# nerfstudio-project/gsplat

Measured on AMD Instinct MI355X. Metric: Mpixels/s fwd+bwd @1M Gaussians/1080p, higher is better.
Workload: dtype f32; 1 GPU; c3: 1M synthetic Gaussians, 1x1920x1080, SH deg 3, 16x16 tiles, fwd+bwd; gaussians_per_gpu=1000000, cameras_per_gpu=1, packed=False, parallelism=single

## Files before the change

gsplat_amd/_autograd.py:

```python
from __future__ import annotations

import torch

from . import _ops

NS = _ops.NS
_registered = False


def _bwd(name):
    return _ops.impl(name + "_bwd")


def _cg(v):
    return None if v is None else v.contiguous()


def _z(v, shape, like):
    return like.new_zeros(shape) if v is None else v


def _qs_setup(ctx, inputs, output):
    quats, scales, compute_covar, compute_preci, triu = inputs
    ctx.triu = triu
    ctx.save_for_backward(quats, scales)


def _qs_backward(ctx, v_covars, v_precis):
    quats, scales = ctx.saved_tensors
    if v_covars is not None and v_covars.is_sparse:
        v_covars = v_covars.to_dense()
    if v_precis is not None and v_precis.is_sparse:
        v_precis = v_precis.to_dense()
    v_quats, v_scales = _bwd("quat_scale_to_covar_preci")(
        quats, scales, ctx.triu,
        None if v_covars is None else v_covars.contiguous(),
        None if v_precis is None else v_precis.contiguous(),
    )
    return v_quats, v_scales, None, None, None


def _sh_setup(ctx, inputs, output):
    (degrees_to_use, means, viewmats, coeffs, masks, batch_ids, camera_ids, gaussian_ids, viewmats_rs) = inputs
    ctx.degrees_to_use = degrees_to_use
    ctx.save_for_backward(means, viewmats, coeffs, masks, batch_ids, camera_ids, gaussian_ids, viewmats_rs)


def _sh_backward(ctx, v_colors):
    means, viewmats, coeffs, masks, batch_ids, camera_ids, gaussian_ids, viewmats_rs = ctx.saved_tensors
    v_coeffs, v_means, v_viewmats, v_viewmats_rs = _bwd("spherical_harmonics")(
        ctx.degrees_to_use, means, viewmats, coeffs, masks, batch_ids, camera_ids, gaussian_ids, viewmats_rs,
        v_colors.contiguous(), ctx.needs_input_grad[1], ctx.needs_input_grad[2],
        len(ctx.needs_input_grad) > 8 and ctx.needs_input_grad[8],
    )
    return (None, v_means, v_viewmats, v_coeffs, None, None, None, None, v_viewmats_rs)


def _proj_setup(ctx, inputs, output):
    (means, covars, quats, scales, _opacities, viewmats, Ks, width, height, eps2d, _near, _far, _clip, _calc,
     camera_model) = inputs
    radii, _means2d, _depths, conics, compensations = output
    ctx.width, ctx.height, ctx.eps2d, ctx.camera_model = width, height, eps2d, camera_model
    ctx.set_materialize_grads(False)
    ctx.m2_shape = _means2d.shape
    ctx.save_for_backward(means, covars, quats, scales, viewmats, Ks, radii, conics, compensations)


def _proj_backward(ctx, v_radii, v_means2d, v_depths, v_conics, v_compensations, v_view_opacities=None):
    means, covars, quats, scales, viewmats, Ks, radii, conics, compensations = ctx.saved_tensors
    if v_compensations is not None:
        v_compensations = v_compensations.contiguous()
    res = _bwd("projection_ewa_3dgs_fused")(
        means, covars, quats, scales, viewmats, Ks, ctx.width, ctx.height, ctx.eps2d, ctx.camera_model, radii, conics,
        compensations, _z(v_means2d, ctx.m2_shape, conics), None if v_depths is None else v_depths.contiguous(),
        _z(v_conics, conics.shape, conics), v_compensations, ctx.needs_input_grad[5], _v_view_opacities=v_view_opacities,
    )
    v_means, v_covars, v_quats, v_scales, v_viewmats = res[:5]
    v_opacities = res[5] if v_view_opacities is not None else None
    if not ctx.needs_input_grad[0]:
        v_means = None
    if not ctx.needs_input_grad[1]:
        v_covars = None
    if not ctx.needs_input_grad[2]:
        v_quats = None
    if not ctx.needs_input_grad[3]:
        v_scales = None
    return (v_means, v_covars, v_quats, v_scales, v_opacities, v_viewmats) + (None,) * 9


class ProjectionWithViewOpacities(torch.autograd.Function):

    @staticmethod
    def forward(ctx, *args):
        with torch._C._AutoDispatchBelowAutograd():
            out = getattr(torch.ops, NS).projection_ewa_3dgs_fused.default(*args)
        _proj_setup(ctx, args, out)
        opacities, viewmats = args[4], args[5]
        per_view = torch.broadcast_to(opacities[..., None, :], opacities.shape[:-1] + (viewmats.shape[-3], opacities.shape[-1]))
        per_view = per_view.contiguous()
        ctx.mark_non_differentiable(out[0])
        return tuple(out) + (per_view,)

    @staticmethod
    def backward(ctx, v_radii, v_means2d, v_depths, v_conics, v_compensations, v_per_view):
        if not ctx.needs_input_grad[4]:
            v_per_view = None
        return _proj_backward(ctx, v_radii, v_means2d, v_depths, v_conics, v_compensations, v_per_view)


def _projp_setup(ctx, inputs, output):
    (means, covars, quats, scales, _opacities, viewmats, Ks, width, height, eps2d, _near, _far, _clip, sparse_grad,
     _calc, camera_model) = inputs
    (batch_ids, camera_ids, gaussian_ids, _indptr, _radii, _means2d, _depths, conics, compensations) = output
    ctx.width, ctx.height, ctx.eps2d, ctx.camera_model, ctx.sparse_grad = width, height, eps2d, camera_model, sparse_grad
    ctx.set_materialize_grads(False)
    ctx.m2_shape = _means2d.shape
    ctx.save_for_backward(means, covars, quats, scales, viewmats, Ks, batch_ids, camera_ids, gaussian_ids, conics,
                          compensations)


def _projp_backward(ctx, v_batch_ids, v_camera_ids, v_gaussian_ids, v_indptr, v_radii, v_means2d, v_depths, v_conics,
                    v_compensations, v_view_opacities=None):
    (means, covars, quats, scales, viewmats, Ks, batch_ids, camera_ids, gaussian_ids, conics,
     compensations) = ctx.saved_tensors
    if v_compensations is not None:
        v_compensations = v_compensations.contiguous()
    res = _bwd("projection_ewa_3dgs_packed")(
        means, covars, quats, scales, viewmats, Ks, ctx.width, ctx.height, ctx.eps2d, ctx.camera_model,
        ctx.sparse_grad, batch_ids, camera_ids, gaussian_ids, conics, compensations,
        _z(v_means2d, ctx.m2_shape, conics), None if v_depths is None else v_depths.contiguous(),
        _z(v_conics, conics.shape, conics), v_compensations, ctx.needs_input_grad[5], _v_view_opacities=v_view_opacities,
    )
    v_means, v_covars, v_quats, v_scales, v_viewmats = res[:5]
    v_opacities = res[5] if v_view_opacities is not None else None
    if not ctx.needs_input_grad[0]:
        v_means = None
    if not ctx.needs_input_grad[1]:
        v_covars = None
    if not ctx.needs_input_grad[2]:
        v_quats = None
    if not ctx.needs_input_grad[3]:
        v_scales = None
    return (v_means, v_covars, v_quats, v_scales, v_opacities, v_viewmats) + (None,) * 10


class PackedProjectionWithViewOpacities(torch.autograd.Function):

    @staticmethod
    def forward(ctx, *args):
        with torch._C._AutoDispatchBelowAutograd():
            out = getattr(torch.ops, NS).projection_ewa_3dgs_packed.default(*args)
        _projp_setup(ctx, args, out)
        opacities = args[4]
        batch_ids, gaussian_ids = out[0], out[2]
        N = opacities.shape[-1]
        flat_ids = gaussian_ids if opacities.dim() == 1 else batch_ids * N + gaussian_ids
        row_opacities = opacities.reshape(-1).index_select(0, flat_ids)
        ctx.mark_non_differentiable(*[t for t in out[:5] if t is not None])
        return tuple(out) + (row_opacities,)

    @staticmethod
    def backward(ctx, v_b, v_c, v_g, v_indptr, v_radii, v_means2d, v_depths, v_conics, v_compensations, v_row_opacities):
        if not ctx.needs_input_grad[4]:
            v_row_opacities = None
        return _projp_backward(ctx, v_b, v_c, v_g, v_indptr, v_radii, v_means2d, v_depths, v_conics, v_compensations,
                               v_row_opacities)


def _rast_setup(ctx, inputs, output):
    (means2d, conics, colors, opacities, backgrounds, masks, image_width, image_height, tile_size, isect_offsets,
     flatten_ids, _packed, absgrad) = inputs
    _render_colors, render_alphas, means2d_absgrad, last_ids = output
    ctx.mark_non_differentiable(last_ids, means2d_absgrad)
    ctx.width, ctx.height, ctx.tile_size, ctx.absgrad = image_width, image_height, tile_size, absgrad
    ctx.set_materialize_grads(False)
    ctx.rc_shape = _render_colors.shape
    ctx.longest = _ops._lookup_longest(flatten_ids)
    ctx.save_for_backward(means2d, conics, colors, opacities, backgrounds, masks, isect_offsets, flatten_ids,
                          render_alphas, last_ids, means2d_absgrad)


def _rast_backward(ctx, v_render_colors, v_render_alphas, v_means2d_absgrad, v_last_ids):
    (means2d, conics, colors, opacities, backgrounds, masks, isect_offsets, flatten_ids, render_alphas, last_ids,
     means2d_absgrad) = ctx.saved_tensors
    v_means2d_abs, v_means2d, v_conics, v_colors, v_opacities, v_backgrounds = _bwd("rasterize_to_pixels_3dgs")(
        means2d, conics, colors, opacities, backgrounds, masks, isect_offsets, flatten_ids, render_alphas, last_ids,
        ctx.width, ctx.height, ctx.tile_size, ctx.absgrad, _z(v_render_colors, ctx.rc_shape, render_alphas),
        None if v_render_alphas is None else v_render_alphas.contiguous(), ctx.needs_input_grad[4], _longest=ctx.longest,
    )
    if ctx.absgrad and v_means2d_abs is not None:
        means2d_absgrad.copy_(v_means2d_abs)
    return (v_means2d, v_conics, v_colors, v_opacities, v_backgrounds) + (None,) * 8


def _rsp_setup(ctx, inputs, output):
    (means2d, conics, colors, opacities, backgrounds, masks, image_ids, image_width, image_height, tile_size, tile_width,
     tile_height, active_tiles, tile_offsets, flatten_ids, tile_pixel_mask, tile_pixel_cumsum, pixel_map, _packed,
     absgrad) = inputs
    _render_colors, render_alphas, means2d_absgrad, last_ids = output
    ctx.mark_non_differentiable(last_ids, means2d_absgrad)
    ctx.geom = (image_width, image_height, tile_size, tile_width, tile_height)
    ctx.absgrad = absgrad
    ctx.set_materialize_grads(False)
    ctx.rc_shape = _render_colors.shape
    ctx.save_for_backward(means2d, conics, colors, opacities, backgrounds, masks, image_ids, active_tiles, tile_offsets,
                          flatten_ids, tile_pixel_mask, tile_pixel_cumsum, pixel_map, render_alphas, last_ids,
                          means2d_absgrad)


def _rsp_backward(ctx, v_render_colors, v_render_alphas, v_means2d_absgrad, v_last_ids):
    (means2d, conics, colors, opacities, backgrounds, masks, image_ids, active_tiles, tile_offsets, flatten_ids,
     tile_pixel_mask, tile_pixel_cumsum, pixel_map, render_alphas, last_ids, means2d_absgrad) = ctx.saved_tensors
    v_means2d_abs, v_means2d, v_conics, v_colors, v_opacities, v_backgrounds = _bwd("rasterize_to_pixels_sparse")(
        means2d, conics, colors, opacities, backgrounds, masks, image_ids, active_tiles, tile_offsets, flatten_ids,
        tile_pixel_mask, tile_pixel_cumsum, pixel_map, render_alphas, last_ids, *ctx.geom, ctx.absgrad,
        _z(v_render_colors, ctx.rc_shape, render_alphas).contiguous(),
        None if v_render_alphas is None else v_render_alphas.contiguous(), ctx.needs_input_grad[4],
    )
    if ctx.absgrad and v_means2d_abs is not None:
        means2d_absgrad.copy_(v_means2d_abs)
    return (v_means2d, v_conics, v_colors, v_opacities, v_backgrounds) + (None,) * 15


def _p2_setup(ctx, inputs, output):
    means, quats, scales, viewmats, Ks, width, height, _eps2d, _near, _far, _clip = inputs
    radii, _means2d, _depths, ray_transforms, _normals = output
    ctx.width, ctx.height = width, height
    ctx.save_for_backward(means, quats, scales, viewmats, Ks, radii, ray_transforms)


def _p2_backward(ctx, v_radii, v_means2d, v_depths, v_ray_transforms, v_normals, v_view_opacities=None):
    means, quats, scales, viewmats, Ks, radii, ray_transforms = ctx.saved_tensors
    res = _bwd("projection_2dgs_fused")(
        means, quats, scales, viewmats, Ks, ctx.width, ctx.height, radii, ray_transforms, v_means2d,
        v_depths, v_ray_transforms, v_normals, ctx.needs_input_grad[3],
        _v_view_opacities=v_view_opacities)
    if v_view_opacities is not None:
        return tuple(res[:4]) + (None,) * 7 + (res[4],)
    return tuple(res) + (None,) * 7


class Projection2DGSWithViewOpacities(torch.autograd.Function):

    @staticmethod
    def forward(ctx, *args):
        op_args, opacities = args[:-1], args[-1]
        with torch._C._AutoDispatchBelowAutograd():
            out = getattr(torch.ops, NS).projection_2dgs_fused.default(*op_args)
        _p2_setup(ctx, op_args, out)
        viewmats = op_args[3]
        per_view = torch.broadcast_to(opacities[..., None, :], opacities.shape[:-1] + (viewmats.shape[-3], opacities.shape[-1]))
        per_view = per_view.contiguous()
        ctx.mark_non_differentiable(out[0])
        return tuple(out) + (per_view,)

    @staticmethod
    def backward(ctx, v_radii, v_means2d, v_depths, v_ray_transforms, v_normals, v_per_view):
        if v_per_view is None or not ctx.needs_input_grad[11]:
            return _p2_backward(ctx, v_radii, v_means2d, v_depths, v_ray_transforms, v_normals) + (None,)
        return _p2_backward(ctx, v_radii, v_means2d, v_depths, v_ray_transforms, v_normals, v_per_view)


def _p2p_setup(ctx, inputs, output):
    means, quats, scales, viewmats, Ks, width, height, _near, _far, _clip, sparse_grad = inputs
    batch_ids, camera_ids, gaussian_ids, _indptr, _radii, _means2d, _depths, ray_transforms, _normals = output
    ctx.width, ctx.height, ctx.sparse_grad = width, height, sparse_grad
    ctx.save_for_backward(means, quats, scales, viewmats, Ks, batch_ids, camera_ids, gaussian_ids, ray_transforms)


def _p2p_backward(ctx, v_b, v_c, v_g, v_indptr, v_radii, v_means2d, v_depths, v_ray_transforms, v_normals):
    means, quats, scales, viewmats, Ks, batch_ids, camera_ids, gaussian_ids, ray_transforms = ctx.saved_tensors
    v_means, v_quats, v_scales, v_viewmats = _bwd("projection_2dgs_packed")(
        means, quats, scales, viewmats, Ks, ctx.width, ctx.height, ctx.sparse_grad, batch_ids, camera_ids,
        gaussian_ids, ray_transforms, v_means2d, v_depths.contiguous(), v_ray_transforms, v_normals,
        ctx.needs_input_grad[3])
    return (v_means, v_quats, v_scales, v_viewmats) + (None,) * 7


def _r2_setup(ctx, inputs, output):
    (means2d, ray_transforms, colors, opacities, normals, densify, backgrounds, masks, image_width, image_height,
     tile_size, tile_offsets, flatten_ids, _packed, absgrad, _distloss) = inputs
    (render_colors, render_alphas, _rn, _rd, _rm, means2d_absgrad, last_ids, median_ids) = output
    ctx.mark_non_differentiable(last_ids, median_ids, means2d_absgrad)
    ctx.width, ctx.height, ctx.tile_size, ctx.absgrad = image_width, image_height, tile_size, absgrad
    ctx.set_materialize_grads(False)
    ctx.rc_shape = render_colors.shape
    ctx.save_for_backward(means2d, ray_transforms, colors, opacities, normals, densify, backgrounds, masks,
                          tile_offsets, flatten_ids, render_colors, render_alphas, last_ids, median_ids,
                          means2d_absgrad)


def _r2_backward(ctx, v_render_colors, v_render_alphas, v_render_normals, v_render_distort, v_render_median,
                 v_absgrad, v_last_ids, v_median_ids):
    (means2d, ray_transforms, colors, opacities, normals, densify, backgrounds, masks, tile_offsets, flatten_ids,
     render_colors, render_alphas, last_ids, median_ids, means2d_absgrad) = ctx.saved_tensors
    (v_means2d_abs, v_means2d, v_ray_transforms, v_colors, v_opacities, v_normals, v_densify,
     v_backgrounds) = _bwd("rasterize_to_pixels_2dgs")(
        means2d, ray_transforms, colors, opacities, normals, densify, backgrounds, masks, tile_offsets, flatten_ids,
        render_colors, render_alphas, last_ids, median_ids, ctx.width, ctx.height, ctx.tile_size, ctx.absgrad,
        _z(v_render_colors, ctx.rc_shape, render_alphas).contiguous(), _cg(v_render_alphas), _cg(v_render_normals),
        _cg(v_render_distort), _cg(v_render_median), ctx.needs_input_grad[6])
    if ctx.absgrad and v_means2d_abs is not None:
        means2d_absgrad.copy_(v_means2d_abs)
    return (v_means2d, v_ray_transforms, v_colors, v_opacities, v_normals, v_densify, v_backgrounds) + (None,) * 9


def _l0_setup(ctx, inputs, output):
    ctx.save_for_backward(inputs[0])


def _l0_backward(ctx, v_colors):
    (sh0,) = ctx.saved_tensors
    return _bwd("spherical_harmonics_l0")(sh0, v_colors.contiguous())


def _l1_setup(ctx, inputs, output):
    (degrees_to_use, means, viewmats, shN, masks, batch_ids, camera_ids, gaussian_ids, viewmats_rs) = inputs
    ctx.degrees_to_use = degrees_to_use
    ctx.save_for_backward(means, viewmats, shN, masks, batch_ids, camera_ids, gaussian_ids, viewmats_rs)


def _l1_backward(ctx, v_colors):
    means, viewmats, shN, masks, batch_ids, camera_ids, gaussian_ids, viewmats_rs = ctx.saved_tensors
    v_shN, v_means, v_viewmats, v_rs = _bwd("spherical_harmonics_l1_plus")(
        ctx.degrees_to_use, means, viewmats, shN, masks, batch_ids, camera_ids, gaussian_ids, viewmats_rs,
        v_colors.contiguous(), ctx.needs_input_grad[1], ctx.needs_input_grad[2],
        len(ctx.needs_input_grad) > 8 and ctx.needs_input_grad[8])
    return (None, v_means, v_viewmats, v_shN, None, None, None, None, v_rs)


def _simple_setup(ctx, inputs, output):
    means, covars, Ks, width, height, camera_model = inputs
    ctx.width, ctx.height, ctx.camera_model = width, height, camera_model
    ctx.save_for_backward(means, covars, Ks)


def _simple_backward(ctx, v_means2d, v_covars2d):
    means, covars, Ks = ctx.saved_tensors
    v_means, v_covars = _bwd("projection_ewa_simple")(means, covars, Ks, ctx.width, ctx.height, ctx.camera_model,
                                                      v_means2d.contiguous(), v_covars2d.contiguous())
    return v_means, v_covars, None, None, None, None


_TABLE = {
    "spherical_harmonics_l0": (_l0_backward, _l0_setup),
    "spherical_harmonics_l1_plus": (_l1_backward, _l1_setup),
    "projection_ewa_simple": (_simple_backward, _simple_setup),
    "projection_2dgs_fused": (_p2_backward, _p2_setup),
    "projection_2dgs_packed": (_p2p_backward, _p2p_setup),
    "rasterize_to_pixels_2dgs": (_r2_backward, _r2_setup),
    "quat_scale_to_covar_preci": (_qs_backward, _qs_setup),
    "spherical_harmonics": (_sh_backward, _sh_setup),
    "projection_ewa_3dgs_fused": (_proj_backward, _proj_setup),
    "projection_ewa_3dgs_packed": (_projp_backward, _projp_setup),
    "rasterize_to_pixels_3dgs": (_rast_backward, _rast_setup),
    "rasterize_to_pixels_sparse": (_rsp_backward, _rsp_setup),
}


def register(extra=None) -> None:
    global _registered
    if _registered:
        return
    table = dict(_TABLE)
    if extra:
        table.update(extra)
    for name, (bwd, setup) in table.items():
        try:
            torch.library.register_autograd(f"{NS}::{name}", bwd, setup_context=setup)
        except RuntimeError as e:
            if "already" not in str(e).lower():
                raise
    _registered = True


register()


class _FastOps:

    def __init__(self, extra=None):
        self._table = dict(_TABLE)
        if extra:
            self._table.update(extra)
        self._ns = getattr(torch.ops, NS)

    def __getattr__(self, name):
        entry = self._table.get(name)
        op = getattr(self._ns, name)
        if entry is None:
            fn = op
        else:
            bwd, setup = entry
            overload = op.default

            class _Fn(torch.autograd.Function):
                @staticmethod
                def forward(ctx, *args):
                    with torch._C._AutoDispatchBelowAutograd():
                        out = overload(*args)
                    setup(ctx, args, out)
                    return out

                @staticmethod
                def backward(ctx, *grads):
                    return bwd(ctx, *grads)

            _Fn.__name__ = _Fn.__qualname__ = f"gsplat_{name}"
            fn = _Fn.apply
        setattr(self, name, fn)
        return fn


fast_ops = _FastOps()
```

gsplat_amd/_cabi.py:

```python
from __future__ import annotations

import ctypes
import json
import os
import threading
from typing import Optional

import torch

_HERE = os.path.dirname(os.path.abspath(__file__))
_LIB_ENV = "GSPLAT_AMD_LIB"


class GsplatAmdError(RuntimeError):
    pass


def lib_path() -> str:
    return os.environ.get(_LIB_ENV) or os.path.join(_HERE, "csrc", "libgsplat_amd.so")


def _load() -> ctypes.CDLL:
    path = lib_path()
    if not os.path.exists(path):
# ... 26 lines not shown
            for a in args.split(","):
                a = " ".join(a.split())
                if "*" in a:
                    codes.append("p")
                elif a.startswith("uint32_t"):
                    codes.append("u")
                elif a.startswith("int64_t"):
                    codes.append("l")
                elif a.startswith("float"):
                    codes.append("f")
                elif a.startswith("double"):
                    codes.append("d")
                elif a.startswith("int "):
                    codes.append("i")
                else:
                    raise ImportError(f"gsplat_amd: cannot parse argument '{a}' of {name} in {path}")
        sigs[name] = ({"int": "i", "int64_t": "l", "void *": "p", "void": "v"}.get(ret, "s"), codes)
    return sigs


_SIG_TABLE = os.path.join(_HERE, "csrc", "abi_signatures.json")


def _load_signatures():
    if os.path.exists(_HEADER):
        return _parse_header(_HEADER)
    if os.path.exists(_SIG_TABLE):
        with open(_SIG_TABLE) as f:
            return {k: (v[0], list(v[1])) for k, v in json.load(f).items()}
    raise ImportError(f"gsplat_amd: neither {_HEADER} nor {_SIG_TABLE} found; rebuild with __graft_entry__.build()")


def write_signature_table() -> str:
    with open(_SIG_TABLE, "w") as f:
        json.dump({k: [v[0], v[1]] for k, v in _parse_header(_HEADER).items()}, f)
    return _SIG_TABLE


SIGNATURES = _load_signatures()


def _bind():
    for name, (ret, codes) in SIGNATURES.items():
        fn = getattr(_lib, name)
        fn.restype = {"i": ctypes.c_int, "l": _L, "s": ctypes.c_char_p, "p": ctypes.c_void_p, "v": None}[ret]
        fn.argtypes = [_CODES[c] for c in codes]


_bind()

ABI_VERSION = _lib.gsx_version()
ARCH = _lib.gsx_arch().decode()


def exported_symbols():
    return list(SIGNATURES)


_tls = threading.local()


def ptr(t: Optional[torch.Tensor]):
    if t is None:
        return None
    if not t.is_cuda:
        raise GsplatAmdError(
            "gsplat_amd kernels only run on a ROCm device (got a CPU tensor); there is no CPU fallback"
        )
    if not t.is_contiguous():
        raise GsplatAmdError("gsplat_amd: tensor must be contiguous")
    _tls.dev = t.device.index
    return t.data_ptr()


def ptr_host(t: torch.Tensor):
    if t.is_cuda or not t.is_pinned():
        raise GsplatAmdError("gsplat_amd: expected a pinned host tensor")
    return t.data_ptr()


def ptr_strided(t: torch.Tensor):
    if not t.is_cuda:
        raise GsplatAmdError("gsplat_amd kernels only run on a ROCm device (got a CPU tensor); there is no CPU fallback")
    _tls.dev = t.device.index
    return t.data_ptr()


_raw_stream = getattr(torch._C, "_cuda_getCurrentRawStream", None)


def current_stream() -> int:
    if _raw_stream is not None:
        return _raw_stream(torch.cuda.current_device())
    return torch.cuda.current_stream().cuda_stream


_profile = None
_profile_only = None


def torch_lib_path() -> str:
    if os.environ.get("GSPLAT_AMD_TORCH_LIB"):
        return os.environ["GSPLAT_AMD_TORCH_LIB"]
    d, base = os.path.split(lib_path())
    if not (base.startswith("libgsplat_amd") and base.endswith(".so")):
        raise ImportError(f"gsplat_amd: {_LIB_ENV}={lib_path()} does not follow the naming rule libgsplat_amd*.so; set "
                          "GSPLAT_AMD_TORCH_LIB to the libgsplat_amd_torch*.so linked against it")
    return os.path.join(d, "libgsplat_amd_torch" + base[len("libgsplat_amd"):])


def check_single_kernel_library() -> None:
    with open("/proc/self/maps") as f:
        libs = {os.path.realpath(ln.split(None, 5)[5].strip()) for ln in f if len(ln.split(None, 5)) == 6}
    kernels = {p for p in libs if os.path.basename(p).startswith("libgsplat_amd") and "_torch" not in os.path.basename(p)}
    if kernels != {os.path.realpath(lib_path())}:
        raise ImportError(f"gsplat_amd: {torch_lib_path()} is linked against {sorted(kernels - {os.path.realpath(lib_path())})}, "
                          f"not {lib_path()}; build the matching torch library (tools/mkvariant.sh, make SUFFIX=... torch)")


_torch_lib = None


def torch_lib() -> ctypes.CDLL:
    global _torch_lib
    if _torch_lib is None:
        lib = ctypes.CDLL(torch_lib_path())
        lib.gsx_torch_seg_len.argtypes, lib.gsx_torch_seg_len.restype = [], ctypes.c_int64
        lib.gsx_torch_profile_begin.argtypes, lib.gsx_torch_profile_begin.restype = [ctypes.c_char_p], None
        lib.gsx_torch_profile_end.restype = ctypes.c_char_p
        _torch_lib = lib
    return _torch_lib


def profile_begin(only=None) -> None:
    global _profile, _profile_only
    _profile = []
    _profile_only = None if only is None else frozenset(only)
    torch_lib().gsx_torch_profile_begin(" ".join(sorted(_profile_only or ())).encode())


def profile_end() -> dict:
    global _profile
    rec, _profile = _profile or [], None
    torch.cuda.synchronize()
    out = {}
    for name, a, b in rec:
        out.setdefault(name, []).append(a.elapsed_time(b))
    for line in torch_lib().gsx_torch_profile_end().decode().splitlines():
        name, ms = line.split()
        out.setdefault(name, []).append(float(ms))
    return out


def call(name: str, *args) -> None:
    dev = getattr(_tls, "dev", None)
    if dev is not None and dev != torch.cuda.current_device():
        _tls.dev = None
        with torch.cuda.device(dev):
            return call(name, *args)
    fn = getattr(_lib, name)
    if _profile is not None and (_profile_only is None or name in _profile_only):
        a, b = torch.cuda.Event(enable_timing=True), torch.cuda.Event(enable_timing=True)
        a.record()
        rc = fn(*args, current_stream())
        b.record()
        _profile.append((name, a, b))
    else:
        rc = fn(*args, current_stream())
    if rc != 0:
        msg = _lib.gsx_last_error().decode(errors="replace")
        if rc == -1:
            raise ValueError(f"{name}: {msg}")
        raise GsplatAmdError(f"{name} failed (code {rc}): {msg}")


def scan_workspace_bytes(n: int) -> int:
    return int(_lib.gsx_scan_workspace_bytes(n))


def sort_workspace_bytes(n: int) -> int:
    return int(_lib.gsx_sort_pairs_workspace_bytes(n))


def appearance_bwd_workspace_floats(n: int, n_cameras: int) -> int:
    return int(_lib.gsx_appearance_bwd_workspace_floats(n, n_cameras))


def knn_workspace_bytes(n: int, k: int) -> int:
    return int(_lib.gsx_knn_workspace_bytes(n, k))


def kmeans_workspace_bytes(n: int, d: int, k: int) -> int:
    return int(_lib.gsx_kmeans_workspace_bytes(n, d, k))


def plas_workspace_bytes(h: int, w: int, c: int) -> int:
    return int(_lib.gsx_plas_workspace_bytes(h, w, c))


def plas_partials_floats(h: int, w: int) -> int:
    return int(_lib.gsx_plas_partials_floats(h, w))


def tile_sort_supported(n_images: int, tile_w: int, tile_h: int) -> bool:
    return bool(_lib.gsx_isect_tile_sort_supported(n_images, tile_w, tile_h))


def tile_sort_workspace_bytes(n: int, n_images: int, tile_w: int, tile_h: int) -> int:
    return int(_lib.gsx_isect_tile_sort_workspace_bytes(n, n_images, tile_w, tile_h))


def isect_fused_supported(n_images: int, tile_w: int, tile_h: int, packed: bool) -> bool:
    return bool(_lib.gsx_isect_fused_supported(n_images, tile_w, tile_h, int(packed)))


class IsectPathMemory:

    def __init__(self):
        self._h = _lib.gsx_isect_path_memory_create()
        if not self._h:
            raise MemoryError("gsx_isect_path_memory_create failed")
        self._prev = []

    def __enter__(self):
        self._prev.append(_lib.gsx_isect_path_memory_use(self._h))
        return self

    def __exit__(self, *exc):
        _lib.gsx_isect_path_memory_use(self._prev.pop())
        return False

    def __del__(self):
        h, self._h = getattr(self, "_h", None), None
        if h:
            _lib.gsx_isect_path_memory_destroy(h)


def copy_column_groups(groups, rows: int) -> None:
    n = len(groups)
    src = (ctypes.c_void_p * n)(*[g[0] for g in groups])
    dst = (ctypes.c_void_p * n)(*[g[2] for g in groups])
    ss = (ctypes.c_uint32 * n)(*[g[1] for g in groups])
    ds = (ctypes.c_uint32 * n)(*[g[3] for g in groups])
    w = (ctypes.c_uint32 * n)(*[g[4] for g in groups])
    call("gsx_copy_column_groups", n, src, ss, dst, ds, w, rows)


def copy_column_groups_mapped(groups, seg_rows, seg_n, map_dst: bool) -> None:
    n, m = len(groups), len(seg_rows)
    src = (ctypes.c_void_p * n)(*[g[0] for g in groups])
    dst = (ctypes.c_void_p * n)(*[g[2] for g in groups])
    ss = (ctypes.c_uint32 * n)(*[g[1] for g in groups])
    ds = (ctypes.c_uint32 * n)(*[g[3] for g in groups])
    w = (ctypes.c_uint32 * n)(*[g[4] for g in groups])
    sr = (ctypes.c_int64 * m)(*[int(v) for v in seg_rows])
    sn = (ctypes.c_int64 * m)(*[int(v) for v in seg_n])
    call("gsx_copy_column_groups_mapped", n, src, ss, dst, ds, w, m, sr, sn, int(bool(map_dst)))


def copy_message_columns(msg_ptr: int, msg_stride: int, rows: int, groups, to_message: bool, seg_rows=None, seg_n=None) -> None:
    n = len(groups)
    cols = (ctypes.c_uint32 * n)(*[g[0] for g in groups])
    w = (ctypes.c_uint32 * n)(*[g[1] for g in groups])
    fields = (ctypes.c_void_p * n)(*[g[2] for g in groups])
    fs = (ctypes.c_uint32 * n)(*[g[3] for g in groups])
    m = 0 if seg_rows is None else len(seg_rows)
    sr = (ctypes.c_int64 * max(m, 1))(*([int(v) for v in seg_rows] if m else [0]))
    sn = (ctypes.c_int64 * max(m, 1))(*([int(v) for v in seg_n] if m else [0]))
    call("gsx_copy_message_columns", ctypes.c_void_p(msg_ptr), msg_stride, rows, n, cols, w, fields, fs, int(bool(to_message)), m,
         sr, sn)


def sort_pairs(keys, vals, keys_alt, vals_alt, n: int, end_bit: int, workspace) -> bool:
    flag = ctypes.c_int(0)
    rc = _lib.gsx_sort_pairs(ptr(keys), ptr(vals), ptr(keys_alt), ptr(vals_alt), n, end_bit, ptr(workspace),
                             workspace.numel() * workspace.element_size(), ctypes.addressof(flag), current_stream())
    if rc != 0:
        raise GsplatAmdError(f"gsx_sort_pairs failed (code {rc}): {_lib.gsx_last_error().decode(errors='replace')}")
    return bool(flag.value)
```

gsplat_amd/_ops.py:

```python
from __future__ import annotations

import math
import os
import threading
from typing import Optional, Tuple

import torch
from torch import Tensor

from . import _cabi
from ._cabi import call, ptr, ptr_strided

NS = "gsplat"

_lib_def = torch.library.Library(NS, "FRAGMENT")
_lib_impl = torch.library.Library(NS, "IMPL", "CUDA")
_lib_impl_autograd = torch.library.Library(NS, "IMPL", "AutogradCUDA")


def _load_torch_lib() -> None:
    path = _cabi.torch_lib_path()
    hint = "build it with `make -C gsplat_amd/csrc torch`"
    if not os.path.exists(path):
        raise ImportError(f"gsplat_amd: {path} not found; {hint}")
# ... 578 lines not shown
         ptr(isect_ids), ptr(flatten_ids))
    if sort:
        isect_ids, flatten_ids = _sort_isects(isect_ids, flatten_ids, I, int(lidar.n_bins_azimuth), int(lidar.n_bins_elevation),
                                              32 + tile_bits + image_bits)
    return tiles_per_gauss, isect_ids, flatten_ids


def _proj_dims(means, viewmats):
    batch_dims = means.shape[:-2]
    return batch_dims, math.prod(batch_dims), viewmats.shape[-3], means.shape[-2]


def _f64_instantiation(fn):
    import functools

    @functools.wraps(fn)
    def body(means, *args, **kw):
        if means.dtype != torch.float64:
            return fn(means, *args, **kw)
        down = lambda t: t.to(torch.float32) if isinstance(t, Tensor) and t.dtype == torch.float64 else t
        up = lambda t: t.to(torch.float64) if isinstance(t, Tensor) and t.dtype == torch.float32 else t
        out = fn(down(means), *[down(a) for a in args], **{k: down(v) for k, v in kw.items()})
        return tuple(up(t) for t in out)

    return body


@_op("projection_ewa_3dgs_fused_bwd")
@_f64_instantiation
def projection_ewa_3dgs_fused_bwd(means, covars, quats, scales, viewmats, Ks, image_width, image_height, eps2d,
                                  camera_model, radii, conics, compensations, v_means2d, v_depths, v_conics,
                                  v_compensations, viewmats_requires_grad, *, _v_view_opacities=None):
    batch_dims, B, C, N = _proj_dims(means, viewmats)
    means, viewmats, Ks = means.contiguous(), viewmats.contiguous(), Ks.contiguous()
    covars, quats, scales = _c(covars), _c(quats), _c(scales)
    v_means = torch.empty_like(means)
    v_covars = v_quats = v_scales = None
    if covars is not None:
        v_covars = torch.empty_like(covars)
    else:
        v_quats, v_scales = torch.empty_like(quats), torch.empty_like(scales)
    v_viewmats = torch.zeros_like(viewmats) if viewmats_requires_grad else None
    v_means2d, m2_stride = _row_view(v_means2d, 2)
    v_conics, con_stride = _row_view(v_conics, 3)
    head = (ptr(means), ptr(covars), ptr(None if covars is not None else quats),
            ptr(None if covars is not None else scales), ptr(viewmats), ptr(Ks), B, C, N, image_width, image_height,
            eps2d, int(camera_model), ptr(radii.contiguous()), ptr(conics.contiguous()), ptr(_c(compensations)),
            ptr_strided(v_means2d), m2_stride, ptr(_c(v_depths)), ptr_strided(v_conics), con_stride,
            ptr(_c(v_compensations)))
    if _v_view_opacities is not None:
        v_view, opac_stride = _elem_view(_v_view_opacities)
        v_opacities = torch.empty(tuple(batch_dims) + (N,), device=means.device, dtype=means.dtype)
        call("gsx_project_ewa_bwd_opac", *head, ptr_strided(v_view), opac_stride, ptr(v_means), ptr(v_covars), ptr(v_quats),
             ptr(v_scales), ptr(v_viewmats), ptr(v_opacities))
        return v_means, v_covars, v_quats, v_scales, v_viewmats, v_opacities
    call("gsx_project_ewa_bwd", *head, ptr(v_means), ptr(v_covars), ptr(v_quats), ptr(v_scales), ptr(v_viewmats))
    return v_means, v_covars, v_quats, v_scales, v_viewmats


@_op("projection_ewa_3dgs_packed_bwd")
@_f64_instantiation
def projection_ewa_3dgs_packed_bwd(means, covars, quats, scales, viewmats, Ks, image_width, image_height, eps2d,
                                   camera_model, sparse_grad, batch_ids, camera_ids, gaussian_ids, conics,
                                   compensations, v_means2d, v_depths, v_conics, v_compensations,
                                   viewmats_requires_grad, *, _v_view_opacities=None):
    batch_dims, B, C, N = _proj_dims(means, viewmats)
    means, viewmats, Ks = means.contiguous(), viewmats.contiguous(), Ks.contiguous()
    covars, quats, scales = _c(covars), _c(quats), _c(scales)
    nnz = gaussian_ids.shape[0]
    v_viewmats = torch.zeros_like(viewmats) if viewmats_requires_grad else None
    v_means2d, m2_stride = _row_view(v_means2d, 2)
    v_conics, con_stride = _row_view(v_conics, 3)
    head = (ptr(means), ptr(covars), ptr(None if covars is not None else quats),
            ptr(None if covars is not None else scales), ptr(viewmats), ptr(Ks), B, C, N, image_width, image_height,
            eps2d, int(camera_model), nnz, ptr(batch_ids.contiguous()), ptr(camera_ids.contiguous()),
            ptr(gaussian_ids.contiguous()), ptr(conics.contiguous()), ptr(_c(compensations)),
            ptr_strided(v_means2d), m2_stride, ptr(_c(v_depths)), ptr_strided(v_conics), con_stride,
            ptr(_c(v_compensations)))
    def scatter_opacities():
        flat = torch.zeros(B * N, device=means.device, dtype=means.dtype)
        flat.index_add_(0, batch_ids * N + gaussian_ids if B > 1 else gaussian_ids, _v_view_opacities.reshape(-1))
        return flat.reshape(tuple(batch_dims) + (N,))

    if sparse_grad:
        def rows(width):
            return torch.empty((nnz, width), device=means.device, dtype=means.dtype)

        r_means = rows(3)
        r_covars = rows(6) if covars is not None else None
        r_quats = rows(4) if covars is None else None
        r_scales = rows(3) if covars is None else None
        call("gsx_project_ewa_packed_bwd_rows", *head, ptr(r_means), ptr(r_covars), ptr(r_quats), ptr(r_scales),
             ptr(v_viewmats))
        flat = len(batch_dims) == 0
        indices = gaussian_ids.unsqueeze(0) if flat else torch.stack([batch_ids, gaussian_ids])
        coalesced = B * C == 1

        def coo(vals, like):
            if vals is None:
                return None
            size = ((N,) if flat else (B, N)) + (like.shape[-1],)
            sp = torch.sparse_coo_tensor(indices, vals, size=size, is_coalesced=coalesced)
            return sp if len(batch_dims) <= 1 else sp.to_dense().reshape(like.shape)

        res = (coo(r_means, means), coo(r_covars, covars), coo(r_quats, quats), coo(r_scales, scales), v_viewmats)
        clear_row_map_cache()
        return res if _v_view_opacities is None else res + (scatter_opacities(),)
    gaussian_major = B * C > 1 or 2 * nnz >= N
    row_map = _packed_row_map(batch_ids, camera_ids, gaussian_ids, B, C, N) if (gaussian_major and nnz > 0 and N > 0) else None
    alloc = torch.empty_like if row_map is not None else torch.zeros_like
    v_means = alloc(means)
    v_covars = v_quats = v_scales = None
    if covars is not None:
        v_covars = alloc(covars)
    else:
        v_quats, v_scales = alloc(quats), alloc(scales)
    v_opacities = None
    if _v_view_opacities is not None:
        v_view, opac_stride = _elem_view(_v_view_opacities)
        v_opacities = (torch.empty if row_map is not None else torch.zeros)(tuple(batch_dims) + (N,), device=means.device, dtype=means.dtype)
        call("gsx_project_ewa_packed_bwd_opac", *head, ptr_strided(v_view), opac_stride, ptr(row_map), ptr(v_means), ptr(v_covars),
             ptr(v_quats), ptr(v_scales), ptr(v_viewmats), ptr(v_opacities))
    else:
        call("gsx_project_ewa_packed_bwd", *head, ptr(row_map), ptr(v_means), ptr(v_covars), ptr(v_quats), ptr(v_scales),
             ptr(v_viewmats))
    clear_row_map_cache()
    res = (v_means, v_covars, v_quats, v_scales, v_viewmats)
    return res if _v_view_opacities is None else res + (v_opacities,)


def _raster_dims(isect_offsets, colors):
    image_dims = tuple(isect_offsets.shape[:-2])
    return image_dims, math.prod(image_dims), isect_offsets.shape[-2], isect_offsets.shape[-1], colors.shape[-1]


def _pixel_linear_strides(t):
    if t.is_contiguous() or t.dim() < 3:
        return None
    shape, stride = t.shape, t.stride()
    cs, ps = stride[-1], stride[-2]
    if cs < 0 or ps < 0:
        return None
    expect = ps
    for d in range(t.dim() - 2, -1, -1):
        if shape[d] != 1 and stride[d] != expect:
            return None
        expect *= shape[d]
    return int(ps), int(cs)


@_op("rasterize_to_pixels_3dgs_bwd")
def rasterize_to_pixels_3dgs_bwd(means2d, conics, colors, opacities, backgrounds, masks, tile_offsets, flatten_ids,
                                 render_alphas, last_ids, image_width, image_height, tile_size, absgrad,
                                 v_render_colors, v_render_alphas, compute_v_backgrounds, *, _longest=None):
    image_dims, I, th, tw, D = _raster_dims(tile_offsets, colors)
    as_received = (means2d, conics, colors, opacities, tile_offsets, flatten_ids)
    means2d, conics, colors, opacities = (means2d.contiguous(), conics.contiguous(), colors.contiguous(),
                                          opacities.contiguous())
    backgrounds, masks = _c(backgrounds), _c(masks)
    v_render_alphas = _c(v_render_alphas)
    R = opacities.numel()
    geo = 8 if absgrad else 6
    longest = _longest if _longest is not None else _lookup_longest(flatten_ids)
    segmented = (longest > SEG_MIN_LONGEST and not absgrad and D <= 4 and tile_size == 16
                 and longest > _seg_cut(flatten_ids.numel(), I, tw, th))
    rows = (torch.zeros if segmented else torch.empty)((R, geo + D), device=means2d.device, dtype=means2d.dtype)
    vrc_strides = None if segmented else _pixel_linear_strides(v_render_colors)
    if vrc_strides is None:
        v_render_colors = v_render_colors.contiguous()
        vrc_strides = (-1, 1)
    if segmented:
        ws = torch.empty(_cabi._lib.gsx_raster3d_bwd_seg_workspace_bytes(flatten_ids.numel(), I, tw, th, D, SEG_LEN),
                         device=means2d.device, dtype=torch.uint8)
        fws = _lookup_seg_workspace(last_ids, flatten_ids.numel(), D, as_received)
        call("gsx_raster3d_bwd_seg_reuse", ptr(means2d), ptr(conics), ptr(colors), ptr(opacities), ptr(backgrounds), ptr(masks),
             ptr(tile_offsets.contiguous()), ptr(flatten_ids.contiguous()), ptr(render_alphas.contiguous()),
             ptr(last_ids.contiguous()), ptr(v_render_colors), ptr(v_render_alphas), I, flatten_ids.numel(), D,
             image_width, image_height, tile_size, tw, th, ptr(rows), geo + D, SEG_LEN, ptr(fws),
             0 if fws is None else fws.numel(), ptr(ws), ws.numel())
    else:
        ws = torch.empty(_cabi._lib.gsx_raster3d_bwd_workspace_bytes(I, tw, th), device=means2d.device, dtype=torch.uint8)
        call("gsx_raster3d_bwd_fill", ptr(means2d), ptr(conics), ptr(colors), ptr(opacities), ptr(backgrounds), ptr(masks),
             ptr(tile_offsets.contiguous()), ptr(flatten_ids.contiguous()), ptr(render_alphas.contiguous()),
             ptr(last_ids.contiguous()), ptr_strided(v_render_colors), ptr(v_render_alphas), I, flatten_ids.numel(), D,
             image_width, image_height, tile_size, tw, th, int(bool(absgrad)), ptr(rows), geo + D, R, vrc_strides[0],
             vrc_strides[1], ptr(ws), ws.numel())
    v_means2d, v_conics = rows[:, 0:2].view(means2d.shape), rows[:, 2:5].view(conics.shape)
    v_opacities, v_colors = rows[:, 5].view(opacities.shape), rows[:, geo:].view(colors.shape)
    v_abs = rows[:, 6:8].view(means2d.shape) if absgrad else None
    v_backgrounds = None
    if backgrounds is not None and compute_v_backgrounds:
        v_backgrounds = (v_render_colors * (1.0 - render_alphas)).sum(dim=(-3, -2))
    return v_abs, v_means2d, v_conics, v_colors, v_opacities, v_backgrounds


_SH_C0 = 0.2820947917738781


@_op("spherical_harmonics_l0")
def spherical_harmonics_l0(sh0):
    if sh0.dim() != 3:
        raise ValueError(f"sh0 must have shape [N, 1, D], got {tuple(sh0.shape)}")
    if sh0.shape[-2] != 1:
        raise ValueError(f"sh0 must contain exactly one SH coefficient, got {tuple(sh0.shape)}")
    if sh0.shape[-1] < 1:
        raise ValueError(f"sh0 last dim D must be >= 1, got {sh0.shape[-1]}")
    if sh0.dtype not in (torch.float32, torch.float16):
        raise TypeError(f"gsplat_amd: sh0 must be float32 or float16 (got {sh0.dtype})")
    return sh0[:, 0, :].float() * _SH_C0


@_op("spherical_harmonics_l0_bwd")
def spherical_harmonics_l0_bwd(sh0, v_colors):
    if v_colors.dim() != 2 or v_colors.shape[0] != sh0.shape[0] or v_colors.shape[1] != sh0.shape[2]:
        raise ValueError(f"v_colors must have shape [N, D], got {tuple(v_colors.shape)}")
    return (v_colors * _SH_C0)[:, None, :].to(sh0.dtype).contiguous()


def _pad_band0(shN):
    return torch.cat([torch.zeros_like(shN[:, :1]), shN], dim=1).contiguous()


_BAND_DTYPES = {torch.float32: 0, torch.float16: 1}


def _sh_band_fwd(degrees_to_use, first_band, means, viewmats, coeffs, masks, batch_ids, camera_ids, gaussian_ids):
    packed, B, C, N, KM, D = _sh_dims(means, viewmats, coeffs, gaussian_ids)
    means, viewmats, coeffs, masks = means.contiguous(), viewmats.contiguous(), coeffs.contiguous(), _c(masks)
    if coeffs.shape[0] != N:
        raise ValueError(f"coefficient rows are indexed by Gaussian: expected {N} rows, got {coeffs.shape[0]}")
    K = KM + first_band
    if packed:
        nnz = gaussian_ids.shape[0]
        colors = torch.empty((nnz, 3), device=means.device, dtype=means.dtype)
        call("gsx_sh_band_fwd", degrees_to_use, first_band, _BAND_DTYPES[coeffs.dtype], ptr(means), ptr(viewmats), ptr(coeffs),
             ptr(masks), ptr(_c(batch_ids)), ptr(_c(camera_ids)), ptr(_c(gaussian_ids)), B, C, N, nnz, K, ptr(colors))
    else:
        colors = torch.empty(viewmats.shape[:-2] + (N, 3), device=means.device, dtype=means.dtype)
        call("gsx_sh_band_fwd", degrees_to_use, first_band, _BAND_DTYPES[coeffs.dtype], ptr(means), ptr(viewmats), ptr(coeffs),
             ptr(masks), None, None, None, B, C, N, -1, K, ptr(colors))
    return colors


def _sh_band_bwd(degrees_to_use, first_band, means, viewmats, coeffs, masks, batch_ids, camera_ids, gaussian_ids, v_colors,
                 compute_v_means, compute_v_viewmats):
    packed, B, C, N, KM, D = _sh_dims(means, viewmats, coeffs, gaussian_ids)
    means, viewmats, coeffs, masks = means.contiguous(), viewmats.contiguous(), coeffs.contiguous(), _c(masks)
    K = KM + first_band
    nnz = gaussian_ids.shape[0] if packed else -1
    row_map = _packed_row_map(batch_ids, camera_ids, gaussian_ids, B, C, N) if (packed and nnz > 0 and N > 0) else None
    if packed and row_map is None:
        return torch.zeros_like(coeffs), (torch.zeros_like(means) if compute_v_means else None), \
            (torch.zeros_like(viewmats) if compute_v_viewmats else None)
    v_coeffs = torch.empty_like(coeffs)
    v_means = torch.empty_like(means) if compute_v_means else None
    v_dirs = None
    if compute_v_viewmats:
        v_dirs = torch.zeros(((nnz if packed else B * C * N), 3), device=means.device, dtype=means.dtype)
    call("gsx_sh_band_bwd", degrees_to_use, first_band, _BAND_DTYPES[coeffs.dtype], ptr(means), ptr(viewmats), ptr(coeffs),
         ptr(masks), B, C, N, nnz, K, ptr(v_colors.contiguous()), ptr(row_map), ptr(v_coeffs), ptr(v_means), ptr(v_dirs))
    v_viewmats = None
    if compute_v_viewmats:
        if packed:
            S = torch.zeros((B * C, 3), device=means.device, dtype=means.dtype)
            S.index_add_(0, batch_ids * C + camera_ids, v_dirs)
        else:
            S = v_dirs.view(B * C, N, 3).sum(dim=1)
        vm = viewmats.reshape(B * C, 4, 4)
        R, t = vm[:, :3, :3], vm[:, :3, 3]
        v_vm = torch.zeros_like(vm)
        v_vm[:, :3, :3] = t[:, :, None] * S[:, None, :]
        v_vm[:, :3, 3] = torch.einsum("cij,cj->ci", R, S)
        v_viewmats = v_vm.reshape(viewmats.shape)
    return v_coeffs, v_means, v_viewmats


def _band_kernels_apply(coeffs) -> bool:
    return coeffs.dim() == 3 and coeffs.shape[-1] == 3 and coeffs.shape[-2] >= 1 and coeffs.dtype in _BAND_DTYPES


@_op("spherical_harmonics_l1_plus")
def spherical_harmonics_l1_plus(degrees_to_use, means, viewmats, shN, masks, batch_ids, camera_ids, gaussian_ids,
                                viewmats_rs=None, *, _gathered: bool = True):
    if viewmats_rs is not None:
        viewmats = _sh_rs_viewmats(viewmats, viewmats_rs)
    if shN.dim() != 3:
        raise ValueError(f"shN must have shape [N, K - 1, D], got {tuple(shN.shape)}")
    _check_sh_inputs(degrees_to_use, means, viewmats, shN, masks, batch_ids, camera_ids, gaussian_ids, omit_l0=True,
                     gathered=_gathered)
    _check_f32(means=means, viewmats=viewmats)
    packed = gaussian_ids is not None
    if degrees_to_use == 0 or shN.shape[-2] == 0:
        shape = (shN.shape[0] if _gathered else gaussian_ids.shape[0], shN.shape[-1]) if packed \
            else tuple(viewmats.shape[:-2]) + (means.shape[-2], shN.shape[-1])
        return torch.zeros(shape, device=means.device, dtype=means.dtype)
    if _band_kernels_apply(shN) and not (packed and _gathered):
        return _sh_band_fwd(degrees_to_use, 1, means, viewmats, shN, masks, batch_ids, camera_ids, gaussian_ids)
    return spherical_harmonics(degrees_to_use, means, viewmats, _pad_band0(shN), masks, batch_ids, camera_ids,
                               gaussian_ids, None, _gathered=_gathered)


@_op("spherical_harmonics_l1_plus_bwd")
def spherical_harmonics_l1_plus_bwd(degrees_to_use, means, viewmats, shN, masks, batch_ids, camera_ids, gaussian_ids,
                                    viewmats_rs, v_colors, compute_v_means, compute_v_viewmats, compute_v_viewmats_rs,
                                    *, _gathered: bool = True):
    if viewmats_rs is not None:
        v_shN, v_me, v_syn, _ = spherical_harmonics_l1_plus_bwd(
            degrees_to_use, means, _sh_rs_viewmats(viewmats, viewmats_rs), shN, masks, batch_ids, camera_ids, gaussian_ids, None,
            v_colors, compute_v_means, compute_v_viewmats or compute_v_viewmats_rs, False, _gathered=_gathered)
        v_vm, v_rs = (None, None) if v_syn is None else _sh_rs_split(v_syn, viewmats, viewmats_rs, compute_v_viewmats,
                                                                     compute_v_viewmats_rs)
        return v_shN, v_me, v_vm, v_rs
    packed = gaussian_ids is not None
    if degrees_to_use == 0 or shN.shape[-2] == 0:
        return (torch.zeros_like(shN), torch.zeros_like(means) if compute_v_means else None,
                torch.zeros_like(viewmats) if compute_v_viewmats else None, None)
    if _band_kernels_apply(shN) and not (packed and _gathered):
        v_shN, v_means, v_viewmats = _sh_band_bwd(degrees_to_use, 1, means, viewmats, shN, masks, batch_ids, camera_ids,
                                                  gaussian_ids, v_colors, compute_v_means, compute_v_viewmats)
        return v_shN, v_means, v_viewmats, None
    v_coeffs, v_means, v_viewmats, v_rs = spherical_harmonics_bwd(
        degrees_to_use, means, viewmats, _pad_band0(shN), masks, batch_ids, camera_ids, gaussian_ids, viewmats_rs,
        v_colors, compute_v_means, compute_v_viewmats, compute_v_viewmats_rs, _gathered=_gathered)
    return v_coeffs[:, 1:].contiguous(), v_means, v_viewmats, v_rs


@_op("projection_ewa_simple")
def projection_ewa_simple(means, covars, Ks, width, height, camera_model):
    _check_f32(means=means, covars=covars, Ks=Ks)
    if means.shape[-1] != 3 or covars.shape[-2:] != (3, 3) or covars.shape[:-2] != means.shape[:-1]:
        raise ValueError(f"proj: bad shapes means {tuple(means.shape)} covars {tuple(covars.shape)}")
    means, covars, Ks = means.contiguous(), covars.contiguous(), Ks.contiguous()
    N = means.shape[-2]
    rows = means.numel() // 3
    means2d = torch.empty(means.shape[:-1] + (2,), device=means.device, dtype=means.dtype)
    covars2d = torch.empty(means.shape[:-1] + (2, 2), device=means.device, dtype=means.dtype)
    call("gsx_project_simple_fwd", ptr(means), ptr(covars), ptr(Ks), rows, N, width, height, int(camera_model),
         ptr(means2d), ptr(covars2d))
    return means2d, covars2d
# ... 1272 lines not shown
```

gsplat_amd/csrc/raster3d.hpp:

```cpp
#pragma once
#include "common.hpp"

#include <type_traits>

namespace gsx {

struct Raster3DArgs {
    uint32_t n_images;
    uint32_t n_isects;
    uint32_t width;
    uint32_t height;
    uint32_t tile_size;
    uint32_t tile_w;
    uint32_t tile_h;
    uint32_t cdim;
    uint32_t ch_off;
    uint32_t nch;
    uint32_t first_chunk;
    const float *means2d;
    const float *conics;
    const float *colors;
    const float *opacities;
    const float *backgrounds;
    const uint8_t *masks;
    const int32_t *isect_offsets;
    const int32_t *flatten_ids;
    float *render_colors;
    float *render_alphas;
    int32_t *last_ids;
    const float *v_render_colors;
    uint32_t vrc_strided;
    int64_t vrc_ps, vrc_cs;
    const float *v_render_alphas;
    float *v_rows;
    uint32_t row_stride;
    const int32_t *sp_active_tiles;
    const uint64_t *sp_pixel_mask;
    const int64_t *sp_pixel_cumsum;
    const int64_t *sp_pixel_map;
    uint32_t n_active, sp_words;
    uint32_t seg_mode, seg_len, seg_grid;
    uint32_t seg_cut;
    const int32_t *seg_items;
    const int32_t *seg_count;
    float *seg_T;
    float *seg_out;
    int32_t *seg_last;
    const int32_t *tile_order;
};

inline Raster3DArgs raster3d_args(uint32_t n_images, uint32_t n_isects, uint32_t cdim, uint32_t width, uint32_t height,
                                  uint32_t tile_size, uint32_t tile_w, uint32_t tile_h, const float *means2d, const float *conics,
                                  const float *colors, const float *opacities, const float *backgrounds, const uint8_t *masks,
                                  const int32_t *isect_offsets, const int32_t *flatten_ids, float *render_colors,
                                  const float *render_alphas, const int32_t *last_ids)
{
    Raster3DArgs a{};
    a.n_images = n_images; a.n_isects = n_isects; a.width = width; a.height = height;
    a.tile_size = tile_size; a.tile_w = tile_w; a.tile_h = tile_h; a.cdim = cdim;
    a.means2d = means2d; a.conics = conics; a.colors = colors; a.opacities = opacities;
    a.backgrounds = backgrounds; a.masks = masks; a.isect_offsets = isect_offsets; a.flatten_ids = flatten_ids;
    a.render_colors = render_colors; a.render_alphas = const_cast<float *>(render_alphas);
    a.last_ids = const_cast<int32_t *>(last_ids);
    return a;
}
inline void raster3d_set_bwd(Raster3DArgs &a, const float *v_render_colors, const float *v_render_alphas, float *v_rows,
                             uint32_t row_stride)
{
    a.v_render_colors = v_render_colors; a.v_render_alphas = v_render_alphas;
    a.v_rows = v_rows; a.row_stride = row_stride;
}
inline void raster3d_set_sparse(Raster3DArgs &a, const int32_t *active_tiles, const uint64_t *tile_pixel_mask,
                                const int64_t *tile_pixel_cumsum, const int64_t *pixel_map, uint32_t n_active,
                                uint32_t words_per_tile)
{
    a.sp_active_tiles = active_tiles; a.sp_pixel_mask = tile_pixel_mask; a.sp_pixel_cumsum = tile_pixel_cumsum;
    a.sp_pixel_map = pixel_map; a.n_active = n_active; a.sp_words = words_per_tile;
}

template <class F>
inline auto with_channels4(uint32_t n, F &&f)
{
    if (n <= 1) return f(std::integral_constant<int, 1>{});
    if (n <= 2) return f(std::integral_constant<int, 2>{});
    if (n <= 3) return f(std::integral_constant<int, 3>{});
    return f(std::integral_constant<int, 4>{});
}
template <class F>
inline auto with_channels(uint32_t n, F &&f)
{
    if (n <= 4) return with_channels4(n, f);
    if (n <= 8) return f(std::integral_constant<int, 8>{});
    if (n <= 16) return f(std::integral_constant<int, 16>{});
    return f(std::integral_constant<int, 32>{});
}

__device__ __forceinline__ uint32_t xcd_remap(uint32_t b, uint32_t n_blocks)
{
    constexpr uint32_t kXcds = 8;
    const uint32_t per_xcd   = (n_blocks + kXcds - 1) / kXcds;
    return (b % kXcds) * per_xcd + (b / kXcds);
}

template <typename Args>
__device__ __forceinline__ size_t vrc_index(const Args &a, size_t pix, uint32_t k)
{
    return a.vrc_strided ? (size_t)((int64_t)pix * a.vrc_ps + (int64_t)k * a.vrc_cs) : pix * a.cdim + k;
}

struct TileCtx {
    uint32_t image_id, tile_id, tile_x, tile_y;
    int32_t range_start, range_end;
};
template <class Args>
__device__ __forceinline__ bool tile_context(const Args &a, uint32_t block, TileCtx &t)
{
    const uint32_t tiles_per_image = a.tile_w * a.tile_h;
    if (a.sp_active_tiles) {
        const uint32_t at = xcd_remap(block, a.n_active);
        if (at >= a.n_active) return false;
        const uint32_t gt = (uint32_t)a.sp_active_tiles[at];
        t.image_id = gt / tiles_per_image;
        t.tile_id  = gt % tiles_per_image;
        t.range_start = a.isect_offsets[at];
        t.range_end   = a.isect_offsets[at + 1];
    } else {
        const uint32_t n_blocks = tiles_per_image * a.n_images;
        const uint32_t blk      = xcd_remap(block, n_blocks);
        if (blk >= n_blocks) return false;
        t.image_id = blk / tiles_per_image;
        t.tile_id  = blk % tiles_per_image;
        t.range_start = a.isect_offsets[blk];
        t.range_end   = (blk == n_blocks - 1) ? (int32_t)a.n_isects : a.isect_offsets[blk + 1];
    }
    t.tile_x = t.tile_id % a.tile_w;
    t.tile_y = t.tile_id / a.tile_w;
    return true;
}
__device__ __forceinline__ bool tile_context_seg(const Raster3DArgs &a, uint32_t block, TileCtx &t, uint32_t &item)
{
    item = 0;
    if (a.seg_mode == 0u) {
        if (!tile_context(a, block, t)) return false;
        return !(a.seg_len && !a.sp_active_tiles && (uint32_t)(t.range_end - t.range_start) > a.seg_cut);
    }
    const int32_t n_items = *a.seg_count;
    const uint32_t tiles_per_image = a.tile_w * a.tile_h, n_blocks = tiles_per_image * a.n_images;
    if ((int32_t)block >= n_items) {
        if (a.seg_mode != 2u) return false;
        const uint32_t blk = block - (uint32_t)n_items;
        if (blk >= n_blocks) return false;
        item       = 0xFFFFFFFFu;
        t.image_id = blk / tiles_per_image;
        t.tile_id  = blk % tiles_per_image;
        t.tile_x   = t.tile_id % a.tile_w;
        t.tile_y   = t.tile_id / a.tile_w;
        t.range_start = a.isect_offsets[blk];
        t.range_end   = (blk == n_blocks - 1) ? (int32_t)a.n_isects : a.isect_offsets[blk + 1];
        return (uint32_t)(t.range_end - t.range_start) <= a.seg_cut;
    }
    item = block;
    const uint32_t blk = (uint32_t)a.seg_items[2 * block];
    t.image_id = blk / tiles_per_image;
    t.tile_id  = blk % tiles_per_image;
    t.tile_x   = t.tile_id % a.tile_w;
    t.tile_y   = t.tile_id / a.tile_w;
    const int32_t tile_end = (blk == n_blocks - 1) ? (int32_t)a.n_isects : a.isect_offsets[blk + 1];
    t.range_start = a.seg_items[2 * block + 1];
    t.range_end   = min(t.range_start + (int32_t)a.seg_len, tile_end);
    return true;
}

template <class Args>
__device__ __forceinline__ int64_t pixel_row(const Args &a, const TileCtx &t, uint32_t block, uint32_t lx, uint32_t ly)
{
    if (!(lx < a.tile_size && ly < a.tile_size)) return -1;
    const uint32_t ox = t.tile_x * a.tile_size + lx, oy = t.tile_y * a.tile_size + ly;
    if (!(ox < a.width && oy < a.height)) return -1;
    if (!a.sp_active_tiles) return ((int64_t)t.image_id * a.height + oy) * a.width + ox;
    const uint32_t at      = xcd_remap(block, a.n_active);
    const uint64_t *words  = a.sp_pixel_mask + (size_t)at * a.sp_words;
    const uint32_t in_tile = ly * a.tile_size + lx, word = in_tile >> 6, bit = in_tile & 63u;
    if (!((words[word] >> bit) & 1ull)) return -1;
    uint32_t rank = __popcll(words[word] & ((1ull << bit) - 1ull));
    for (uint32_t w = 0; w < word; ++w) rank += __popcll(words[w]);
    const int64_t first = at == 0 ? 0 : a.sp_pixel_cumsum[at - 1];
    return a.sp_pixel_map[first + rank];
}

int64_t tile_order_workspace_bytes(uint32_t n_images, uint32_t tile_w, uint32_t tile_h);
const int32_t *build_tile_order(const int32_t *isect_offsets, const int32_t *last_ids, uint32_t n_images, uint32_t tile_size,
                                uint32_t tile_w, uint32_t tile_h, uint32_t width, uint32_t height, uint32_t n_isects, void *ws,
                                int64_t ws_bytes, hipStream_t stream, int *rc, void *zero_ptr = nullptr, int64_t zero_bytes = 0);

struct RowFill {
    const char *fn;
    float *rows;
    int64_t bytes;
    hipStream_t stream;
    template <class Args>
    const int32_t *tile_order(const Args &a, void *ws, int64_t ws_bytes, int *rc)
    {
        const bool in_kernel = bytes > 0 && (reinterpret_cast<uintptr_t>(rows) & 15u) == 0;
        const int32_t *order = build_tile_order(a.isect_offsets, a.last_ids, a.n_images, a.tile_size, a.tile_w, a.tile_h, a.width,
                                                a.height, a.n_isects, ws, ws_bytes, stream, rc, in_kernel ? rows : nullptr, bytes);
        if (*rc == GSX_OK && order && in_kernel) bytes = 0;
        return order;
    }
    int now()
    {
        if (bytes > 0 && rows && hipMemsetAsync(rows, 0, (size_t)bytes, stream) != hipSuccess) {
            set_last_error("%s: memset failed", fn);
            return GSX_ERR_LAUNCH;
        }
        bytes = 0;
        return GSX_OK;
    }
};

bool raster3d_fwd_m_applies(const Raster3DArgs &a);
int raster3d_fwd_m_launch(const Raster3DArgs &a, hipStream_t stream);

__device__ __forceinline__ bool tile_context_ordered(const Raster3DArgs &a, uint32_t block, TileCtx &t)
{
    const uint32_t tiles_per_image = a.tile_w * a.tile_h, n_blocks = tiles_per_image * a.n_images;
    const uint32_t idx = xcd_remap(block, n_blocks);
    if (idx >= n_blocks) return false;
    const uint32_t blk = (uint32_t)a.tile_order[idx];
    t.image_id = blk / tiles_per_image;
    t.tile_id  = blk % tiles_per_image;
    t.tile_x   = t.tile_id % a.tile_w;
    t.tile_y   = t.tile_id / a.tile_w;
    t.range_start = a.isect_offsets[blk];
    t.range_end   = (blk == n_blocks - 1) ? (int32_t)a.n_isects : a.isect_offsets[blk + 1];
    return true;
}

enum class BwdKernel { R, T, W, M };
BwdKernel raster3d_bwd_kernel(uint32_t tile_size, uint32_t nch, bool has_abs);
int raster3d_bwd_m_launch(const Raster3DArgs &a, hipStream_t stream);

__device__ __forceinline__ void tile_pixel(uint32_t tid, uint32_t tile_size, uint32_t &lx, uint32_t &ly)
{
    if (tile_size == 16) {
        const uint32_t w = tid >> 6, l = tid & 63u;
        lx = ((w & 1u) << 3) | (l & 7u);
        ly = ((w >> 1) << 3) | (l >> 3);
    } else {
        lx = tid % tile_size;
        ly = tid / tile_size;
    }
}

constexpr float kLog2e = 1.4426950408889634f;
__device__ __forceinline__ void stage_gaussian(float x, float y, float opac, float ca, float cb, float cc, float4 &ga,
                                               float2 &gb)
{
    const float lo = opac > 0.0f ? __log2f(opac) : -INFINITY;
    ga = make_float4(x, y, lo, 0.5f * kLog2e * ca);
    gb = make_float2(kLog2e * cb, 0.5f * kLog2e * cc);
}
__device__ __forceinline__ float staged_q(const float4 &ga, const float2 &gb, float dx, float dy)
{
    return fmaf(dx, fmaf(ga.w, dx, gb.x * dy), gb.y * dy * dy);
}
__device__ __forceinline__ float staged_alpha_raw(const float4 &ga, float q)
{
    return __builtin_amdgcn_exp2f(ga.z - q);
}
__device__ __forceinline__ float staged_e_offset(const float4 &ga, const float2 &gb, float dx, float dy)
{
    return fmaf(dx, fmaf(-gb.x, dy, -ga.w * dx), fmaf(-gb.y * dy, dy, ga.z));
}

struct StagedRow {
    v4f p0;
    v4f p1;
    v4f p2;
};
__device__ __forceinline__ void stage_gaussian_f(float ax, float ay, float opac, float ca, float cb, float cc, v4f &p0,
                                                 float &nA, float &nB, float &nC)
{
    const float lo = opac > 0.0f ? __log2f(opac) : -INFINITY;
    p0 = v4f{ax, ay, lo, lo};
    nA = -0.5f * kLog2e * ca; nB = -kLog2e * cb; nC = -0.5f * kLog2e * cc;
}
__device__ __forceinline__ float staged_f(const v4f &p0, float nA, float nB, float nC, float u, float v)
{
    const float dx = p0.x - u, dy = p0.y - v;
    return fmaf(dx, fmaf(nB, dy, nA * dx), fmaf(nC * dy, dy, p0.z));
}

__device__ __forceinline__ float2 cull_half_extent(float opac, float ca, float cb, float cc)
{
    const float L   = __logf(255.0f * opac) + 0.01f;
    const float det = ca * cc - cb * cb;
    if (!(det > 0.0f)) return make_float2(INFINITY, INFINITY);
    if (!(L > 0.0f)) return make_float2(-1.0f, -1.0f);
    const float k = 2.0f * L / det;
    return make_float2(sqrtf(k * cc) * 1.0001f + 1e-3f, sqrtf(k * ca) * 1.0001f + 1e-3f);
}

struct WaveRect {
    float cx, cy, hw, hh;
    bool any;
};
__device__ __forceinline__ WaveRect wave_pixel_rect(bool inside, float px, float py)
{
    float xmin = inside ? px : INFINITY, xmax = inside ? px : -INFINITY;
    float ymin = inside ? py : INFINITY, ymax = inside ? py : -INFINITY;
#pragma unroll
    for (int o = 32; o >= 1; o >>= 1) {
        xmin = fminf(xmin, __shfl_xor(xmin, o));
        xmax = fmaxf(xmax, __shfl_xor(xmax, o));
        ymin = fminf(ymin, __shfl_xor(ymin, o));
        ymax = fmaxf(ymax, __shfl_xor(ymax, o));
    }
    WaveRect r;
    r.any = xmin <= xmax;
    r.cx = 0.5f * (xmin + xmax); r.hw = 0.5f * (xmax - xmin);
    r.cy = 0.5f * (ymin + ymax); r.hh = 0.5f * (ymax - ymin);
    return r;
}

__device__ __forceinline__ bool rect_reaches_level(const v4f &p0, const v4f &p1, float ax, float ay, const WaveRect &r)
{
    const float A = -p1.x, B = -p1.y, C = -p1.z;
    if (!(A > 0.0f && C > 0.0f && 4.0f * A * C > B * B)) return true;
    const float dxl = ax - r.cx - r.hw, dxh = ax - r.cx + r.hw, dyl = ay - r.cy - r.hh, dyh = ay - r.cy + r.hh;
    const float dxe = fminf(fmaxf(0.0f, dxl), dxh), dye = fminf(fmaxf(0.0f, dyl), dyh);
    const float dys = fminf(fmaxf(-0.5f * B * dxe * __builtin_amdgcn_rcpf(C), dyl), dyh);
    const float dxs = fminf(fmaxf(-0.5f * B * dye * __builtin_amdgcn_rcpf(A), dxl), dxh);
    const float q1 = fmaf(dxe, fmaf(A, dxe, B * dys), C * dys * dys);
    const float q2 = fmaf(dxs, fmaf(A, dxs, B * dye), C * dye * dye);
    return fminf(q1, q2) <= p0.w + (7.99435344f + 0.01f);
}

}
```

gsplat_amd/csrc/raster3d_bwd.hip:

```cpp
#include <cstdlib>

#include "raster3d.hpp"
#include "../../include/gsplat_amd.h"

namespace gsx {

template <int CH, bool ABS>
struct BwdCfg {
    static constexpr int K     = CH + 6 + (ABS ? 2 : 0);
    static constexpr bool TAIL1 = (K % 4) == 1;
    static constexpr int KQ    = TAIL1 ? K / 4 : (K + 3) / 4;
    static constexpr int KP    = (K | 1);
    static constexpr int BATCH = (CH >= 16) ? 128 : 256;
    static constexpr size_t smem =
        (size_t)BATCH * (2 * sizeof(float4) + sizeof(float2) + sizeof(int32_t) * 2 + sizeof(float) * (CH + KP));
};

template <int CH, bool ABS>
__global__ void __launch_bounds__(256) raster3d_bwd_kernel(const Raster3DArgs a)
{
    using Cfg           = BwdCfg<CH, ABS>;
    constexpr int K     = Cfg::K;
    constexpr int KQ    = Cfg::KQ;
    constexpr int KP    = Cfg::KP;
// ... 827 lines not shown
                contributed |= 1 << q;
            }
            if (contributed) {
                const int info = (t << 4) | contributed;
                uint32_t m0_saved;
                asm("s_mov_b32 %1, m0\n\ts_mov_b32 m0, %3\n\tv_writelane_b32 %0, %2, m0\n\ts_mov_b32 m0, %1"
                    : "+v"(slot_info), "=&s"(m0_saved)
                    : "s"(info), "s"(slot));
                w_ptr += SP;
                if (++slot == SLOTS) {
                    turn(SLOTS);
                    slot  = 0;
                    w_ptr = w_ptr0;
                }
            }
        }
        if (slot) {
            turn(slot);
            slot  = 0;
            w_ptr = w_ptr0;
        }
    }
}

template <int CH>
__global__ void __launch_bounds__(64) __attribute__((amdgpu_waves_per_eu(GSX_BWD_W_WAVES)))
raster3d_bwd_w_kernel(Raster3DArgs a)
{
    raster3d_bwd_w_body<CH, false>(a);
}
__global__ void __launch_bounds__(64) __attribute__((amdgpu_waves_per_eu(2))) raster3d_bwd_w4_kernel(Raster3DArgs a)
{
    raster3d_bwd_w_body<4, false>(a);
}
template <int CH>
__global__ void __launch_bounds__(64) __attribute__((amdgpu_waves_per_eu(GSX_BWD_W_ABS_WAVES)))
raster3d_bwd_w_abs_kernel(Raster3DArgs a)
{
    raster3d_bwd_w_body<CH, true>(a);
}

BwdKernel raster3d_bwd_kernel(uint32_t tile_size, uint32_t nch, bool has_abs)
{
    static const char v = [] {
        const char *e = getenv("GSX_RASTER3D_BWD");
        if (e && (e[0] == 'r' || e[0] == 'R')) return 'r';
        if (e && (e[0] == 't' || e[0] == 'T')) return 't';
        return 'w';
    }();
    if (tile_size != 16 || v == 'r') return BwdKernel::R;
    if (nch > 4) return !has_abs && nch <= 32 ? BwdKernel::M : BwdKernel::R;
    if (v == 'w') return BwdKernel::W;
    return has_abs ? BwdKernel::R : BwdKernel::T;
}

template <int CH, bool ABS>
static int launch_bwd(const Raster3DArgs &a, BwdKernel kernel, hipStream_t stream)
{
    const uint32_t n_blocks = a.sp_active_tiles ? a.n_active : a.tile_w * a.tile_h * a.n_images;
    if (n_blocks == 0 || a.n_isects == 0) return GSX_OK;
    const uint32_t grid  = ((n_blocks + 7u) / 8u) * 8u;
    if constexpr (CH <= 4) {
        if (kernel == BwdKernel::W) {
            if constexpr (ABS) raster3d_bwd_w_abs_kernel<CH><<<dim3(grid), dim3(64), BwdWCfg<CH, true>::smem, stream>>>(a);
            else if constexpr (CH == 4) raster3d_bwd_w4_kernel<<<dim3(grid), dim3(64), BwdWCfg<4>::smem, stream>>>(a);
            else raster3d_bwd_w_kernel<CH><<<dim3(grid), dim3(64), BwdWCfg<CH>::smem, stream>>>(a);
            return check_launch("raster3d_bwd_w");
        }
        if constexpr (!ABS) {
            if (kernel == BwdKernel::T) {
                raster3d_bwd_t_kernel<CH><<<dim3(grid), dim3(256), BwdTCfg<CH>::smem, stream>>>(a);
                return check_launch("raster3d_bwd_t");
            }
        }
    }
    const uint32_t block = a.tile_size <= 8 ? 64u : 256u;
    using Cfg = BwdCfg<CH, ABS>;
    const size_t smem = Cfg::smem;
    raster3d_bwd_kernel<CH, ABS><<<dim3(grid), dim3(block), smem, stream>>>(a);
    return check_launch("raster3d_bwd");
}

int raster3d_bwd_t_launch_items(const Raster3DArgs &a, hipStream_t stream)
{
    const uint32_t grid = ((a.seg_grid + 7u) / 8u) * 8u;
    if (grid == 0) return GSX_OK;
    with_channels4(a.nch, [&](auto ch) {
        raster3d_bwd_t_kernel<ch()><<<dim3(grid), dim3(256), BwdTCfg<ch()>::smem, stream>>>(a);
    });
    return check_launch("raster3d_bwd_t(segments)");
}
template <bool ABS>
static int bwd_dispatch(Raster3DArgs a, hipStream_t stream)
{
    uint32_t off = 0;
    bool first   = true;
    do {
        const uint32_t rem = a.cdim - off;
        const uint32_t n   = rem > 32 ? 32 : rem;
        a.ch_off           = off;
        a.nch              = n;
        a.first_chunk      = first ? 1u : 0u;
        const BwdKernel kernel = raster3d_bwd_kernel(a.tile_size, n, ABS);
        const int rc           = kernel == BwdKernel::M ? raster3d_bwd_m_launch(a, stream)
                                                        : with_channels(n, [&](auto ch) { return launch_bwd<ch(), ABS>(a, kernel, stream); });
        if (rc != GSX_OK) return rc;
        off += n;
        first = false;
    } while (off < a.cdim);
    return GSX_OK;
}

}

extern "C" int64_t gsx_raster3d_bwd_workspace_bytes(uint32_t n_images, uint32_t tile_w, uint32_t tile_h)
{
    return gsx::tile_order_workspace_bytes(n_images, tile_w, tile_h);
}

extern "C" int gsx_raster3d_bwd(
    const float *means2d, const float *conics, const float *colors, const float *opacities,
    const float *backgrounds, const uint8_t *masks, const int32_t *isect_offsets, const int32_t *flatten_ids,
    const float *render_alphas, const int32_t *last_ids, const float *v_render_colors, const float *v_render_alphas,
    uint32_t n_images, uint32_t n_isects, uint32_t cdim, uint32_t width, uint32_t height, uint32_t tile_size,
    uint32_t tile_w, uint32_t tile_h, int has_abs, float *v_rows, uint32_t row_stride, void *stream)
{
    return gsx_raster3d_bwd_ws(means2d, conics, colors, opacities, backgrounds, masks, isect_offsets, flatten_ids, render_alphas,
                               last_ids, v_render_colors, v_render_alphas, n_images, n_isects, cdim, width, height, tile_size,
                               tile_w, tile_h, has_abs, v_rows, row_stride, -1, 1, nullptr, 0, stream);
}

extern "C" int gsx_raster3d_bwd_ws(
    const float *means2d, const float *conics, const float *colors, const float *opacities,
    const float *backgrounds, const uint8_t *masks, const int32_t *isect_offsets, const int32_t *flatten_ids,
    const float *render_alphas, const int32_t *last_ids, const float *v_render_colors, const float *v_render_alphas,
    uint32_t n_images, uint32_t n_isects, uint32_t cdim, uint32_t width, uint32_t height, uint32_t tile_size,
    uint32_t tile_w, uint32_t tile_h, int has_abs, float *v_rows, uint32_t row_stride, int64_t v_colors_pixel_stride,
    int64_t v_colors_channel_stride, void *workspace, int64_t workspace_bytes, void *stream)
{
    return gsx_raster3d_bwd_fill(means2d, conics, colors, opacities, backgrounds, masks, isect_offsets, flatten_ids, render_alphas,
                                 last_ids, v_render_colors, v_render_alphas, n_images, n_isects, cdim, width, height, tile_size,
                                 tile_w, tile_h, has_abs, v_rows, row_stride, 0, v_colors_pixel_stride, v_colors_channel_stride,
                                 workspace, workspace_bytes, stream);
}

extern "C" int gsx_raster3d_bwd_fill(
    const float *means2d, const float *conics, const float *colors, const float *opacities,
    const float *backgrounds, const uint8_t *masks, const int32_t *isect_offsets, const int32_t *flatten_ids,
    const float *render_alphas, const int32_t *last_ids, const float *v_render_colors, const float *v_render_alphas,
    uint32_t n_images, uint32_t n_isects, uint32_t cdim, uint32_t width, uint32_t height, uint32_t tile_size,
    uint32_t tile_w, uint32_t tile_h, int has_abs, float *v_rows, uint32_t row_stride, int64_t v_rows_to_fill,
    int64_t v_colors_pixel_stride, int64_t v_colors_channel_stride, void *workspace, int64_t workspace_bytes, void *stream)
{
    using namespace gsx;
    RowFill fill{"gsx_raster3d_bwd_fill", v_rows, v_rows_to_fill > 0 ? v_rows_to_fill * (int64_t)row_stride * 4 : 0,
                 (hipStream_t)stream};
    GSX_REQUIRE(tile_size >= 1 && tile_size <= 16, "gsx_raster3d_bwd: tile_size must be in [1,16], got %u", tile_size);
    GSX_REQUIRE(cdim >= 1, "gsx_raster3d_bwd: channels must be >= 1");
    if (n_isects == 0) return fill.now();
    GSX_REQUIRE(v_rows, "gsx_raster3d_bwd: null gradient output");
    GSX_REQUIRE(row_stride >= 6u + (has_abs ? 2u : 0u) + cdim,
                "gsx_raster3d_bwd: row_stride %u too small for 6%s + %u channels", row_stride, has_abs ? " + 2" : "", cdim);
    GSX_REQUIRE(n_isects == 0 || (means2d && conics && colors && opacities && flatten_ids && render_alphas && last_ids
                                  && v_render_colors && isect_offsets),
                "gsx_raster3d_bwd: null input");
    Raster3DArgs a = raster3d_args(n_images, n_isects, cdim, width, height, tile_size, tile_w, tile_h, means2d, conics, colors,
                                   opacities, backgrounds, masks, isect_offsets, flatten_ids, nullptr, render_alphas, last_ids);
    raster3d_set_bwd(a, v_render_colors, v_render_alphas, v_rows, row_stride);
    if (v_colors_pixel_stride >= 0) {
        GSX_REQUIRE(v_colors_channel_stride >= 0, "gsx_raster3d_bwd_ws: negative channel stride");
        a.vrc_strided = 1u; a.vrc_ps = v_colors_pixel_stride; a.vrc_cs = v_colors_channel_stride;
    }
    if (raster3d_bwd_kernel(tile_size, cdim > 32 ? 32 : cdim, has_abs != 0) != BwdKernel::R) {
        int rc       = GSX_OK;
        a.tile_order = fill.tile_order(a, workspace, workspace_bytes, &rc);
        if (rc != GSX_OK) return rc;
    }
    if (int rc = fill.now(); rc != GSX_OK) return rc;
    return has_abs ? bwd_dispatch<true>(a, (hipStream_t)stream) : bwd_dispatch<false>(a, (hipStream_t)stream);
}

extern "C" int gsx_raster3d_sparse_bwd(
    const float *means2d, const float *conics, const float *colors, const float *opacities, const float *backgrounds,
    const uint8_t *masks, const int32_t *active_tiles, const int32_t *tile_offsets, const int32_t *flatten_ids,
    const uint64_t *tile_pixel_mask, const int64_t *tile_pixel_cumsum, const int64_t *pixel_map, uint32_t n_active,
    uint32_t words_per_tile, const float *render_alphas, const int32_t *last_ids, const float *v_render_colors,
    const float *v_render_alphas, uint32_t n_images, uint32_t n_isects, uint32_t cdim, uint32_t width, uint32_t height,
    uint32_t tile_size, uint32_t tile_w, uint32_t tile_h, int has_abs, float *v_rows, uint32_t row_stride, void *stream)
{
    using namespace gsx;
    GSX_REQUIRE(tile_size >= 1 && tile_size <= 16, "gsx_raster3d_sparse_bwd: tile_size must be in [1,16], got %u", tile_size);
    GSX_REQUIRE(cdim >= 1, "gsx_raster3d_sparse_bwd: channels must be >= 1");
    if (n_isects == 0) return GSX_OK;
    GSX_REQUIRE(v_rows, "gsx_raster3d_sparse_bwd: null gradient output");
    GSX_REQUIRE(row_stride >= 6u + (has_abs ? 2u : 0u) + cdim, "gsx_raster3d_sparse_bwd: row_stride %u too small", row_stride);
    if (n_active == 0 || n_isects == 0) return GSX_OK;
    GSX_REQUIRE(words_per_tile * 64u >= tile_size * tile_size, "gsx_raster3d_sparse_bwd: pixel mask too narrow");
    GSX_REQUIRE(active_tiles && tile_offsets && tile_pixel_mask && tile_pixel_cumsum && pixel_map && means2d && conics
                && colors && opacities && flatten_ids && render_alphas && last_ids && v_render_colors,
                "gsx_raster3d_sparse_bwd: null input");
    Raster3DArgs a = raster3d_args(n_images, n_isects, cdim, width, height, tile_size, tile_w, tile_h, means2d, conics, colors,
                                   opacities, backgrounds, masks, tile_offsets, flatten_ids, nullptr, render_alphas, last_ids);
    raster3d_set_bwd(a, v_render_colors, v_render_alphas, v_rows, row_stride);
    raster3d_set_sparse(a, active_tiles, tile_pixel_mask, tile_pixel_cumsum, pixel_map, n_active, words_per_tile);
    return has_abs ? bwd_dispatch<true>(a, (hipStream_t)stream) : bwd_dispatch<false>(a, (hipStream_t)stream);
}
```

gsplat_amd/csrc/raster3d_fwd.hip:

```cpp
#include "raster3d.hpp"
#include "../../include/gsplat_amd.h"

namespace gsx {

constexpr int kBatch = 256;


template <int CH, bool PRE = false>
__global__ void __launch_bounds__(256) raster3d_fwd_kernel(const Raster3DArgs a)
{
    extern __shared__ __attribute__((aligned(16))) unsigned char smem_raw[];
    constexpr int CX = CH > 4 ? CH - 4 : 0;
    StagedRow *s_st = reinterpret_cast<StagedRow *>(smem_raw);
    float4 *s_cull  = reinterpret_cast<float4 *>(s_st + kBatch);
    float *s_col    = reinterpret_cast<float *>(s_cull + kBatch);

    TileCtx tc;
    uint32_t seg_item;
    if (!tile_context_seg(a, blockIdx.x, tc, seg_item)) return;
    const uint32_t seg_mode = seg_item == 0xFFFFFFFFu ? 0u : a.seg_mode;
    const uint32_t tiles_per_image = a.tile_w * a.tile_h;
    const uint32_t image_id = tc.image_id, tile_id = tc.tile_id;
    const uint32_t tid      = threadIdx.x;

    uint32_t lx, ly;
    tile_pixel(tid, a.tile_size, lx, ly);
    const int64_t prow = pixel_row(a, tc, blockIdx.x, lx, ly);
    const bool inside  = prow >= 0;
    const float half = 0.5f * (float)a.tile_size;
    const float cx   = (float)(tc.tile_x * a.tile_size) + half, cy = (float)(tc.tile_y * a.tile_size) + half;
    const float u    = (float)lx + 0.5f - half, v = (float)ly + 0.5f - half;
    const size_t pix = inside ? (size_t)prow : 0;

    const float *bg = a.backgrounds ? a.backgrounds + (size_t)image_id * a.cdim + a.ch_off : nullptr;

    if (a.masks && !a.masks[(size_t)image_id * tiles_per_image + tile_id]) {
        if constexpr (PRE) {
            a.seg_T[(size_t)seg_item * 256 + tid]   = 1.0f;
            a.seg_out[(size_t)seg_item * 256 + tid] = 0.0f;
            return;
        }
        if (seg_mode == 1u) {
            a.seg_T[(size_t)seg_item * 256 + tid] = 1.0f;
            return;
        }
        if (seg_mode == 2u) {
            for (uint32_t k = 0; k < a.nch; ++k) a.seg_out[((size_t)seg_item * (a.nch + 1) + k) * 256 + tid] = 0.0f;
            a.seg_out[((size_t)seg_item * (a.nch + 1) + a.nch) * 256 + tid] = 1.0f;
            a.seg_last[(size_t)seg_item * 256 + tid] = -1;
            return;
        }
        if (inside) {
#pragma unroll
            for (int k = 0; k < CH; ++k)
                if (k < (int)a.nch) a.render_colors[pix * a.cdim + a.ch_off + k] = bg ? bg[k] : 0.0f;
            if (a.first_chunk) {
                a.render_alphas[pix] = 0.0f;
                a.last_ids[pix]      = 0;
            }
        }
        return;
    }

    const int32_t range_start = tc.range_start;
    int32_t range_end = tc.range_end;
    int32_t last_id   = -1;
    if constexpr (PRE) {
        last_id = inside ? a.last_ids[pix] : -1;
        __shared__ int32_t s_m[4];
        const int32_t wm = wave_max_i32(last_id);
        if ((tid & 63u) == 0) s_m[tid >> 6] = wm;
        __syncthreads();
        range_end = min(range_end, max(max(s_m[0], s_m[1]), max(s_m[2], s_m[3])) + 1);
    }
    const int32_t n_batches = range_end > range_start ? (range_end - range_start + kBatch - 1) / kBatch : 0;

    float T          = 1.0f;
    uint32_t cur_idx = seg_mode ? 0xFFFFFFFFu : 0u;
    float acc[CH];
#pragma unroll
    for (int k = 0; k < CH; ++k) acc[k] = 0.0f;
    float thr = inside ? kAlphaThreshold : INFINITY;
    if (seg_mode == 2u) {
        T = a.seg_T[(size_t)seg_item * 256 + tid];
        if (!(T > kTransmittanceThresh)) thr = INFINITY;
    }
    const uint32_t lane = tid & 63u;

    for (int32_t b = 0; b < n_batches; ++b) {
        if (__syncthreads_count(!(thr < INFINITY)) == (int)blockDim.x) break;

        const int32_t batch_start = __builtin_amdgcn_readfirstlane(range_start + kBatch * b);
        for (int s = (int)tid; s < kBatch; s += (int)blockDim.x) {
            const int32_t idx = batch_start + s;
            if (idx < range_end) {
                const int32_t g  = a.flatten_ids[idx];
                const float2 xy  = reinterpret_cast<const float2 *>(a.means2d)[g];
                const float opac = a.opacities[g];
                const float ca = a.conics[3 * (size_t)g], cb = a.conics[3 * (size_t)g + 1], cc = a.conics[3 * (size_t)g + 2];
                const float ax = xy.x - cx, ay = xy.y - cy;
                v4f p0;
                float nA, nB, nC;
                stage_gaussian_f(ax, ay, opac, ca, cb, cc, p0, nA, nB, nC);
                const float2 he = cull_half_extent(opac, ca, cb, cc);
                s_cull[s]       = make_float4(ax, ay, he.x, he.y);
                const float *c  = a.colors + (size_t)g * a.cdim + a.ch_off;
                float cv[CH > 4 ? CH : 4];
#pragma unroll
                for (int k = 0; k < (CH > 4 ? CH : 4); ++k) cv[k] = (k < CH && k < (int)a.nch) ? c[k] : 0.0f;
                s_st[s].p0 = p0;
                s_st[s].p1 = v4f{nA, nB, nC, cv[2]};
                s_st[s].p2 = v4f{cv[0], cv[1], cv[3], 0.0f};
#pragma unroll
                for (int k = 4; k < CH; ++k) s_col[s * CX + k - 4] = cv[k];
            }
        }
        __syncthreads();

        const int32_t batch_size = min(kBatch, range_end - batch_start);
        const WaveRect rect = wave_pixel_rect(thr < INFINITY, u, v);
        for (int32_t j = 0; j < batch_size; j += 64) {
            if (__builtin_amdgcn_ballot_w64(thr < INFINITY) == 0ull) break;
            const int32_t tl = j + (int32_t)lane;
            bool hit         = false;
            if (tl < batch_size) {
                const float4 cu = s_cull[tl];
                hit = (fabsf(cu.x - rect.cx) - rect.hw <= cu.z) && (fabsf(cu.y - rect.cy) - rect.hh <= cu.w);
                if (hit) hit = rect_reaches_level(s_st[tl].p0, s_st[tl].p1, cu.x, cu.y, rect);
            }
            uint64_t todo = __builtin_amdgcn_ballot_w64(hit);
            while (todo) {
                const int32_t bit = (int32_t)__builtin_ctzll(todo);
                const int32_t t   = j + bit;
                asm("s_bitset0_b64 %0, %1" : "+s"(todo) : "s"(bit));

                const v4f p0 = s_st[t].p0;
                const v4f p1 = s_st[t].p1;
                const v4f p2 = s_st[t].p2;
                const float e     = staged_f(p0, p1.x, p1.y, p1.z, u, v);
                const float alpha = fminf(kMaxAlpha, __builtin_amdgcn_exp2f(e));
                bool ok = !(e > p0.w) && !(alpha < thr);
                if constexpr (PRE) ok = ok && (batch_start + t <= last_id);
                if (__builtin_amdgcn_ballot_w64(ok) == 0ull) continue;
                const float next_T = fmaf(-T, alpha, T);
                const bool low     = PRE ? false : next_T <= kTransmittanceThresh;
                const bool sat = ok && low, take = ok && !sat;
                const float at = take ? alpha : 0.0f;
                const float w  = at * T;
                acc[0] += p2.x * w;
                if constexpr (CH > 1) acc[1] += p2.y * w;
                if constexpr (CH > 2) acc[2] += p1.w * w;
                if constexpr (CH > 3) acc[3] += p2.z * w;
#pragma unroll
                for (int k = 4; k < CH; ++k) acc[k] += s_col[t * CX + k - 4] * w;
                cur_idx = take ? (uint32_t)(batch_start + t) : cur_idx;
                T       = fmaf(-T, at, T);
                thr     = sat ? INFINITY : thr;
            }
        }
    }

    if constexpr (PRE) {
        float S = 0.0f;
        if (inside) {
#pragma unroll
            for (int k = 0; k < CH; ++k)
                if (k < (int)a.nch) S = fmaf(acc[k], a.v_render_colors[pix * a.cdim + a.ch_off + k], S);
        }
        a.seg_T[(size_t)seg_item * 256 + tid]   = T;
        a.seg_out[(size_t)seg_item * 256 + tid] = S;
        return;
    }
    if (seg_mode == 1u) {
        a.seg_T[(size_t)seg_item * 256 + tid] = (inside && !(thr < INFINITY)) ? 0.0f : T;
        return;
    }
    if (seg_mode == 2u) {
#pragma unroll
        for (int k = 0; k < CH; ++k)
            if (k < (int)a.nch) a.seg_out[((size_t)seg_item * (a.nch + 1) + k) * 256 + tid] = acc[k];
        a.seg_out[((size_t)seg_item * (a.nch + 1) + a.nch) * 256 + tid] = T;
        a.seg_last[(size_t)seg_item * 256 + tid] = (int32_t)cur_idx;
        return;
    }
    if (inside) {
#pragma unroll
        for (int k = 0; k < CH; ++k)
            if (k < (int)a.nch)
                a.render_colors[pix * a.cdim + a.ch_off + k] = bg ? (acc[k] + T * bg[k]) : acc[k];
        if (a.first_chunk) {
            a.render_alphas[pix] = 1.0f - T;
            a.last_ids[pix]      = (int32_t)cur_idx;
        }
    }
}

template <int CH>
static int launch_fwd(const Raster3DArgs &a, hipStream_t stream)
{
    const uint32_t n_blocks = a.seg_mode ? a.seg_grid : (a.sp_active_tiles ? a.n_active : a.tile_w * a.tile_h * a.n_images);
    if (n_blocks == 0) return GSX_OK;
    const uint32_t grid   = ((n_blocks + 7u) / 8u) * 8u;
    const uint32_t block  = a.tile_size <= 8 ? 64u : 256u;
    const size_t smem     = kBatch * (sizeof(StagedRow) + sizeof(float4) + sizeof(float) * (CH > 4 ? CH - 4 : 0));
    hipLaunchKernelGGL(raster3d_fwd_kernel<CH>, dim3(grid), dim3(block), smem, stream, a);
    return check_launch("raster3d_fwd");
}

int raster3d_bwd_prepass_launch(const Raster3DArgs &a, hipStream_t stream)
{
    const uint32_t grid = ((a.seg_grid + 7u) / 8u) * 8u;
    if (grid == 0) return GSX_OK;
    const size_t smem = kBatch * (sizeof(StagedRow) + sizeof(float4));
    with_channels4(a.nch, [&](auto ch) {
        hipLaunchKernelGGL((raster3d_fwd_kernel<ch(), true>), dim3(grid), dim3(256), smem, stream, a);
    });
    return check_launch("raster3d_bwd_prepass");
}

int raster3d_fwd_launch_chunk(const Raster3DArgs &a, hipStream_t stream)
{
    if (raster3d_fwd_m_applies(a)) return raster3d_fwd_m_launch(a, stream);
    return with_channels(a.nch, [&](auto ch) { return launch_fwd<ch()>(a, stream); });
}

int raster3d_fwd_dispatch(Raster3DArgs a, hipStream_t stream)
{
    uint32_t off = 0;
    bool first   = true;
    do {
        const uint32_t rem = a.cdim - off;
        const uint32_t n   = rem > 32 ? 32 : rem;
        a.ch_off           = off;
        a.nch              = n;
        a.first_chunk      = first ? 1u : 0u;
        const int rc = raster3d_fwd_launch_chunk(a, stream);
        if (rc != GSX_OK) return rc;
        off += n;
        first = false;
    } while (off < a.cdim);
    return GSX_OK;
}

}

extern "C" int gsx_raster3d_fwd(
    const float *means2d, const float *conics, const float *colors, const float *opacities,
    const float *backgrounds, const uint8_t *masks, const int32_t *isect_offsets, const int32_t *flatten_ids,
    uint32_t n_images, uint32_t n_isects, uint32_t cdim, uint32_t width, uint32_t height, uint32_t tile_size,
    uint32_t tile_w, uint32_t tile_h, float *render_colors, float *render_alphas, int32_t *last_ids, void *stream)
{
    using namespace gsx;
    GSX_REQUIRE(tile_size >= 1 && tile_size <= 16, "gsx_raster3d_fwd: tile_size must be in [1,16], got %u", tile_size);
    GSX_REQUIRE(cdim >= 1, "gsx_raster3d_fwd: channels must be >= 1");
    GSX_REQUIRE(render_colors && render_alphas && last_ids, "gsx_raster3d_fwd: null output");
    GSX_REQUIRE(n_isects == 0 || (means2d && conics && colors && opacities && flatten_ids),
                "gsx_raster3d_fwd: null input");
    GSX_REQUIRE(isect_offsets != nullptr || n_images * tile_w * tile_h == 0, "gsx_raster3d_fwd: null isect_offsets");
    Raster3DArgs a = raster3d_args(n_images, n_isects, cdim, width, height, tile_size, tile_w, tile_h, means2d, conics, colors,
                                   opacities, backgrounds, masks, isect_offsets, flatten_ids, render_colors, render_alphas, last_ids);
    return raster3d_fwd_dispatch(a, (hipStream_t)stream);
}

extern "C" int gsx_raster3d_sparse_fwd(
    const float *means2d, const float *conics, const float *colors, const float *opacities, const float *backgrounds,
    const uint8_t *masks, const int32_t *active_tiles, const int32_t *tile_offsets, const int32_t *flatten_ids,
    const uint64_t *tile_pixel_mask, const int64_t *tile_pixel_cumsum, const int64_t *pixel_map, uint32_t n_active,
    uint32_t words_per_tile, uint32_t n_images, uint32_t n_isects, uint32_t cdim, uint32_t width, uint32_t height,
    uint32_t tile_size, uint32_t tile_w, uint32_t tile_h, float *render_colors, float *render_alphas, int32_t *last_ids,
    void *stream)
{
    using namespace gsx;
    GSX_REQUIRE(tile_size >= 1 && tile_size <= 16, "gsx_raster3d_sparse_fwd: tile_size must be in [1,16], got %u", tile_size);
    GSX_REQUIRE(cdim >= 1, "gsx_raster3d_sparse_fwd: channels must be >= 1");
    if (n_active == 0) return GSX_OK;
    GSX_REQUIRE(words_per_tile * 64u >= tile_size * tile_size, "gsx_raster3d_sparse_fwd: pixel mask too narrow");
    GSX_REQUIRE(active_tiles && tile_offsets && tile_pixel_mask && tile_pixel_cumsum && pixel_map && render_colors
                && render_alphas && last_ids, "gsx_raster3d_sparse_fwd: null layout / output");
    GSX_REQUIRE(n_isects == 0 || (means2d && conics && colors && opacities && flatten_ids), "gsx_raster3d_sparse_fwd: null input");
    Raster3DArgs a = raster3d_args(n_images, n_isects, cdim, width, height, tile_size, tile_w, tile_h, means2d, conics, colors,
                                   opacities, backgrounds, masks, tile_offsets, flatten_ids, render_colors, render_alphas, last_ids);
    raster3d_set_sparse(a, active_tiles, tile_pixel_mask, tile_pixel_cumsum, pixel_map, n_active, words_per_tile);
    return raster3d_fwd_dispatch(a, (hipStream_t)stream);
}
```

gsplat_amd/csrc/tile_order.hip:

```cpp
#include <cstdlib>

#include "raster3d.hpp"

namespace gsx {

constexpr uint32_t kOrderBuckets = 1024;
struct TileOrderArgs {
    const int32_t *isect_offsets, *last_ids;
    uint32_t n_images, tile_w, tile_h, width, height, n_isects, n_blocks, per_xcd;
    int32_t *cost;
    int32_t *order;
    void *zero_ptr;
    int64_t zero_bytes;
};
__global__ void __launch_bounds__(256) tile_order_cost_kernel(const TileOrderArgs a)
{
    if (a.zero_ptr) {
        const int64_t n16 = a.zero_bytes >> 4;
        uint4 *z          = reinterpret_cast<uint4 *>(a.zero_ptr);
        for (int64_t i = (int64_t)blockIdx.x * 256 + threadIdx.x; i < n16; i += (int64_t)gridDim.x * 256) z[i] = make_uint4(0u, 0u, 0u, 0u);
        if (blockIdx.x == 0 && (int64_t)threadIdx.x < ((a.zero_bytes & 15) >> 2))
            reinterpret_cast<float *>(a.zero_ptr)[n16 * 4 + threadIdx.x] = 0.0f;
    }
    const uint32_t lane = threadIdx.x & 63u, blk = blockIdx.x * 4u + (threadIdx.x >> 6);
    if (blk >= a.n_blocks) return;
    const uint32_t tiles_per_image = a.tile_w * a.tile_h;
    const uint32_t image = blk / tiles_per_image, tile = blk % tiles_per_image;
    const uint32_t x0 = (tile % a.tile_w) * 16u, y0 = (tile / a.tile_w) * 16u;
    int32_t m = -1;
#pragma unroll
    for (uint32_t i = 0; i < 4; ++i) {
        const uint32_t p = lane + 64u * i, ox = x0 + (p & 15u), oy = y0 + (p >> 4);
        if (ox < a.width && oy < a.height) m = max(m, a.last_ids[((size_t)image * a.height + oy) * a.width + ox]);
    }
    m = wave_max_i32(m);
    if (lane == 0) {
        const int32_t start = a.isect_offsets[blk];
        const int32_t end   = (blk == a.n_blocks - 1) ? (int32_t)a.n_isects : a.isect_offsets[blk + 1];
        a.cost[blk]         = max(0, min(end, m + 1) - start);
    }
}
__global__ void __launch_bounds__(1024) tile_order_sort_kernel(const TileOrderArgs a)
{
    __shared__ int32_t s_hist[kOrderBuckets];
    __shared__ int32_t s_wave[16];
    const uint32_t tid = threadIdx.x, lane = tid & 63u, wave = tid >> 6;
    const uint32_t first = blockIdx.x * a.per_xcd, last = min(first + a.per_xcd, a.n_blocks);
    s_hist[tid] = 0;
    __syncthreads();
    for (uint32_t blk = first + tid; blk < last; blk += 1024u)
        atomicAdd(&s_hist[min((uint32_t)a.cost[blk] >> 2, kOrderBuckets - 1u)], 1);
    __syncthreads();
    const int32_t mine = s_hist[kOrderBuckets - 1u - tid];
    int32_t inc        = mine;
#pragma unroll
    for (int o = 1; o < 64; o <<= 1) {
        const int32_t y = __shfl_up(inc, o);
        if ((int)lane >= o) inc += y;
    }
    if (lane == 63u) s_wave[wave] = inc;
    __syncthreads();
    int32_t before = 0;
    for (uint32_t w = 0; w < wave; ++w) before += s_wave[w];
    s_hist[kOrderBuckets - 1u - tid] = before + inc - mine;
    __syncthreads();
    for (uint32_t blk = first + tid; blk < last; blk += 1024u) {
        const int32_t slot = atomicAdd(&s_hist[min((uint32_t)a.cost[blk] >> 2, kOrderBuckets - 1u)], 1);
        a.order[first + (uint32_t)slot] = (int32_t)blk;
    }
}

}

namespace gsx {

static int bwd_lpt_mode()
{
    static const int mode = [] {
        const char *e = getenv("GSX_RASTER3D_BWD_ORDER");
        if (e && (e[0] == '0' || e[0] == 'l')) return 0;
        if (e && e[0] == 'f') return 2;
        return 1;
    }();
    return mode;
}
const int32_t *build_tile_order(const int32_t *isect_offsets, const int32_t *last_ids, uint32_t n_images, uint32_t tile_size,
                                uint32_t tile_w, uint32_t tile_h, uint32_t width, uint32_t height, uint32_t n_isects, void *ws,
                                int64_t ws_bytes, hipStream_t stream, int *rc, void *zero_ptr, int64_t zero_bytes)
{
    *rc = GSX_OK;
    const uint32_t n_blocks = tile_w * tile_h * n_images;
    const int mode = bwd_lpt_mode();
    if (!ws || tile_size != 16 || mode == 0 || (mode == 1 && n_blocks < 2048u)) return nullptr;
    if (ws_bytes < tile_order_workspace_bytes(n_images, tile_w, tile_h)) return nullptr;
    TileOrderArgs o{};
    o.isect_offsets = isect_offsets; o.last_ids = last_ids; o.n_images = n_images; o.tile_w = tile_w; o.tile_h = tile_h;
    o.width = width; o.height = height; o.n_isects = n_isects; o.n_blocks = n_blocks; o.per_xcd = (n_blocks + 7u) / 8u;
    o.cost  = reinterpret_cast<int32_t *>(ws);
    o.order = o.cost + n_blocks;
    o.zero_ptr = zero_ptr; o.zero_bytes = zero_bytes;
    tile_order_cost_kernel<<<dim3((n_blocks + 3u) / 4u), dim3(256), 0, stream>>>(o);
    tile_order_sort_kernel<<<dim3((n_blocks + o.per_xcd - 1u) / o.per_xcd), dim3(1024), 0, stream>>>(o);
    *rc = check_launch("tile order");
    return *rc == GSX_OK ? o.order : nullptr;
}


int64_t tile_order_workspace_bytes(uint32_t n_images, uint32_t tile_w, uint32_t tile_h)
{
    return (int64_t)sizeof(int32_t) * 2ll * n_images * tile_w * tile_h;
}

}
```

gsplat_amd/csrc/torch_ops.cpp:

```cpp
#include <chrono>
#include <cstdlib>
#include <thread>
#include <ATen/ATen.h>
#include <ATen/hip/impl/HIPStreamMasqueradingAsCUDA.h>
#include <c10/core/DeviceGuard.h>
#include <torch/library.h>

#include <hip/hip_runtime_api.h>

#include <algorithm>
#include <atomic>
#include <cmath>
#include <mutex>
#include <set>
#include <string>
#include <tuple>
#include <vector>

#include "../../include/gsplat_amd.h"

namespace gsplat_amd {
namespace {

using at::Tensor;
// ... 199 lines not shown
    }
    const int64_t nnz = wait_nnz();
    auto o = outputs(nnz);
    if (nnz > 0 || true) write(nnz, o);
    return o;
}
struct TensorKey {
    std::optional<c10::weak_intrusive_ptr<c10::StorageImpl>> storage;
    int64_t offset = 0, n = 0;
    TensorKey() = default;
    explicit TensorKey(const Tensor &t)
    {
        if (!t.defined() || t.numel() <= 0 || !t.has_storage()) return;
        storage = c10::weak_intrusive_ptr<c10::StorageImpl>(
            c10::intrusive_ptr<c10::StorageImpl>::reclaim_copy(t.storage().unsafeGetStorageImpl()));
        offset = t.storage_offset(); n = t.numel();
    }
    const c10::StorageImpl *target() const { return storage ? storage->_unsafe_get_target() : nullptr; }
    bool expired() const { return storage && storage->expired(); }
    bool same_storage(const Tensor &t) const
    {
        return storage && t.defined() && t.has_storage() && target() == t.storage().unsafeGetStorageImpl();
    }
    bool matches(const Tensor &t) const { return same_storage(t) && offset == t.storage_offset() && n == t.numel(); }
};
static std::atomic<uint64_t> g_note_seq{0};
template <class Note, size_t N> Note &note_slot(Note (&table)[N], const Tensor &t)
{
    Note *pick = nullptr;
    for (auto &e : table)
        if (e.key.same_storage(t)) return e;
    for (auto &e : table)
        if (!e.key.storage || e.key.expired()) return e;
    for (auto &e : table)
        if (!pick || e.seq < pick->seq) pick = &e;
    return *pick;
}

struct LongestNote {
    TensorKey key;
    uint64_t seq = 0;
    int64_t longest = 0;
};
static std::mutex g_notes_mu;
static LongestNote g_notes[16];
void note_longest(const Tensor &flat, int64_t longest)
{
    TensorKey key(flat);
    if (!key.storage) return;
    std::lock_guard<std::mutex> lock(g_notes_mu);
    note_slot(g_notes, flat) = LongestNote{std::move(key), ++g_note_seq, longest};
}
int64_t lookup_longest(const Tensor &flat)
{
    std::lock_guard<std::mutex> lock(g_notes_mu);
    for (const auto &e : g_notes)
        if (e.key.matches(flat)) return e.longest;
    return 0;
}

struct SegWsNote {
    TensorKey key;
    uint64_t seq = 0;
    int64_t n_isects = 0, cdim = 0, seg_len = 0;
    std::vector<std::pair<TensorKey, int64_t>> inputs;
    Tensor ws;
    bool made_from(at::TensorList ts) const
    {
        if (ts.size() != inputs.size()) return false;
        for (size_t i = 0; i < inputs.size(); ++i)
            if (!inputs[i].first.matches(ts[i]) || inputs[i].second != tensor_version(ts[i])) return false;
        return true;
    }
    static int64_t tensor_version(const Tensor &t) { return t.defined() && !t.is_inference() ? (int64_t)t._version() : 0; }
};
static std::mutex g_seg_ws_mu;
static SegWsNote g_seg_ws[4];
static void seg_ws_purge_locked()
{
    for (auto &e : g_seg_ws)
        if (e.key.expired()) e = SegWsNote();
}
void note_seg_workspace(const Tensor &last_ids, const Tensor &ws, int64_t n_isects, int64_t cdim, int64_t seg_len,
                        at::TensorList inputs)
{
    SegWsNote fresh;
    fresh.key = TensorKey(last_ids);
    if (!fresh.key.storage) return;
    fresh.n_isects = n_isects; fresh.cdim = cdim; fresh.seg_len = seg_len; fresh.ws = ws;
    for (const Tensor &t : inputs) fresh.inputs.emplace_back(TensorKey(t), SegWsNote::tensor_version(t));
    std::lock_guard<std::mutex> lock(g_seg_ws_mu);
    seg_ws_purge_locked();
    fresh.seq = ++g_note_seq;
    note_slot(g_seg_ws, last_ids) = std::move(fresh);
}
OptTensor lookup_seg_workspace(const Tensor &last_ids, int64_t n_isects, int64_t cdim, int64_t seg_len, at::TensorList inputs)
{
    std::lock_guard<std::mutex> lock(g_seg_ws_mu);
    seg_ws_purge_locked();
    for (const auto &e : g_seg_ws)
        if (e.key.matches(last_ids) && e.made_from(inputs) && e.n_isects == n_isects && e.cdim == cdim && e.seg_len == seg_len
            && e.ws.defined() && e.ws.device() == last_ids.device())
            return e.ws;
    return std::nullopt;
}
static bool seg_reuse_env()
{
    static const bool v = [] {
        const char *e = std::getenv("GSPLAT_AMD_SEG_REUSE");
        return !(e && (e[0] == '0' || e[0] == 0));
    }();
    return v;
}

Tensor bytes(int64_t n, const Tensor &like) { return at::empty({n < 8 ? 8 : n}, like.options().dtype(at::kByte)); }

Tensor intersect_offset(const Tensor &isect_ids_, int64_t I, int64_t tile_w, int64_t tile_h)
{
    Launch L(isect_ids_);
    const Tensor ids = contig(isect_ids_);
    Tensor offsets = at::empty({I, tile_h, tile_w}, ids.options().dtype(at::kInt));
    { Timed timed_("gsx_isect_offsets", L.stream); check(gsx_isect_offsets(cp<int64_t>(ids), ids.numel(), (uint32_t)I, (uint32_t)tile_w, (uint32_t)tile_h, mp<int32_t>(offsets),
                            L.stream),
          "gsx_isect_offsets"); }
    return offsets;
}

struct RasterDims {
    std::vector<int64_t> image_dims;
    int64_t I, th, tw, D;
};
RasterDims raster_dims(const Tensor &isect_offsets, const Tensor &colors)
{
    RasterDims r;
    r.image_dims.assign(isect_offsets.sizes().begin(), isect_offsets.sizes().end() - 2);
    r.I = prod(r.image_dims);
    r.th = isect_offsets.size(-2);
    r.tw = isect_offsets.size(-1);
    r.D = colors.size(-1);
    return r;
}

static int64_t seg_len_env()
{
    static const int64_t v = [] {
        const char *e = std::getenv("GSPLAT_AMD_SEG_LEN");
        return e ? (int64_t)std::atoll(e) : (int64_t)768;
    }();
    return v;
}
#define kSegLen (seg_len_env())

std::tuple<Tensor, Tensor, Tensor, Tensor>
rasterize_to_pixels_3dgs(const Tensor &means2d_, const Tensor &conics_, const Tensor &colors_, const Tensor &opacities_,
                         const OptTensor &backgrounds_, const OptTensor &masks_, int64_t width, int64_t height, int64_t tile_size,
                         const Tensor &isect_offsets_, const Tensor &flatten_ids_, bool packed, bool absgrad)
{
    (void)packed;
    want_f32(means2d_, "means2d"); want_f32(conics_, "conics"); want_f32(colors_, "colors"); want_f32(opacities_, "opacities");
    want_f32(backgrounds_, "backgrounds");
    Launch L(means2d_);
    const RasterDims r = raster_dims(isect_offsets_, colors_);
    TORCH_CHECK(r.th * tile_size >= height && r.tw * tile_size >= width,
                      "rasterize_to_pixels: isect_offsets tile grid does not cover the image");
    TORCH_CHECK(!has(masks_) || masks_->scalar_type() == at::kBool, "masks must be a bool tensor");
    const Tensor means2d = contig(means2d_), conics = contig(conics_), colors = contig(colors_), opac = contig(opacities_);
    const OptTensor bg = contig(backgrounds_), masks = contig(masks_);
    const Tensor offsets = contig(isect_offsets_), flat = contig(flatten_ids_);
    auto shape = [&](std::initializer_list<int64_t> tail) {
        auto s = r.image_dims;
        s.insert(s.end(), tail);
        return s;
    };
    Tensor renders = at::empty(shape({height, width, r.D}), means2d.options());
    Tensor alphas = at::empty(shape({height, width, 1}), means2d.options());
    Tensor last_ids = at::empty(shape({height, width}), means2d.options().dtype(at::kInt));
    const int64_t longest = lookup_longest(flatten_ids_);
    if (kSegLen > 0 && longest > gsx_raster3d_seg_cut(flat.numel(), (uint32_t)r.I, (uint32_t)r.tw, (uint32_t)r.th, (uint32_t)kSegLen)) {
        Tensor ws = at::empty({gsx_raster3d_seg_workspace_bytes(flat.numel(), (uint32_t)r.I, (uint32_t)r.tw, (uint32_t)r.th, (uint32_t)r.D,
                                                              (uint32_t)kSegLen)}, means2d.options().dtype(at::kByte));
        Timed timed_("gsx_raster3d_fwd", L.stream);
        check(gsx_raster3d_fwd_seg(fp(means2d), fp(conics), fp(colors), fp(opac), fp(bg),
                                   masks ? (const uint8_t *)masks->const_data_ptr<bool>() : nullptr, cp<int32_t>(offsets),
                                   cp<int32_t>(flat), (uint32_t)r.I, (uint32_t)flat.numel(), (uint32_t)r.D, (uint32_t)width,
                                   (uint32_t)height, (uint32_t)tile_size, (uint32_t)r.tw, (uint32_t)r.th, mp<float>(renders),
                                   mp<float>(alphas), mp<int32_t>(last_ids), (uint32_t)kSegLen, ws.mutable_data_ptr(), ws.numel(), L.stream),
              "gsx_raster3d_fwd_seg");
        if (r.D <= 4 && tile_size == 16 && seg_reuse_env())
            note_seg_workspace(last_ids, ws, flat.numel(), r.D, kSegLen, {means2d_, conics_, colors_, opacities_, isect_offsets_, flatten_ids_});
    } else { Timed timed_("gsx_raster3d_fwd", L.stream); check(gsx_raster3d_fwd(fp(means2d), fp(conics), fp(colors), fp(opac), fp(bg),
                           masks ? (const uint8_t *)masks->const_data_ptr<bool>() : nullptr, cp<int32_t>(offsets),
                           cp<int32_t>(flat), (uint32_t)r.I, (uint32_t)flat.numel(), (uint32_t)r.D, (uint32_t)width,
                           (uint32_t)height, (uint32_t)tile_size, (uint32_t)r.tw, (uint32_t)r.th, mp<float>(renders),
                           mp<float>(alphas), mp<int32_t>(last_ids), L.stream),
          "gsx_raster3d_fwd"); }
    Tensor holder = absgrad ? at::zeros_like(means2d) : at::empty({0}, means2d.options());
    return {renders, alphas, holder, last_ids};
}

const uint8_t *mask_ptr(const OptTensor &m) { return has(m) && m->numel() ? (const uint8_t *)m->const_data_ptr<bool>() : nullptr; }

std::tuple<OptTensor, Tensor, Tensor, Tensor>
isect_fused_begin(const Tensor &means2d, const Tensor &radii, const Tensor &depths, const OptTensor &conics, const OptTensor &opac,
                  const OptTensor &tile_mask, int64_t rows, int64_t I, int64_t tile_size, int64_t tile_w, int64_t tile_h, c10::IntArrayRef out_shape)
{
    Launch L(means2d);
    const uint32_t uI = (uint32_t)I, uts = (uint32_t)tile_size, utw = (uint32_t)tile_w, uth = (uint32_t)tile_h;
    TORCH_CHECK(!has(tile_mask) || (tile_mask->scalar_type() == at::kBool && tile_mask->is_contiguous()
                                    && tile_mask->numel() == I * tile_w * tile_h),
                "isect_fused_begin: tile_mask must be a contiguous bool tensor of n_images * tiles flags");
    Tensor tiles_per_gauss;
    if (!out_shape.empty()) tiles_per_gauss = at::empty(out_shape, means2d.options().dtype(at::kInt));
    auto result = [&](const Tensor &offsets, const Tensor &count_ws, const Tensor &host_total) {
        return std::make_tuple(tiles_per_gauss.defined() ? OptTensor(tiles_per_gauss) : OptTensor(), offsets, count_ws, host_total);
    };
    Tensor host_total = at::empty({3}, at::TensorOptions().dtype(at::kLong).pinned_memory(true));
    host_total.mutable_data_ptr<int64_t>()[0] = -1;
    host_total.mutable_data_ptr<int64_t>()[1] = 0;
    const bool binned_path = gsx_isect_binned_should_try(rows, uI, utw, uth, 0) != 0;
    host_total.mutable_data_ptr<int64_t>()[2] = binned_path ? 1 : 0;
    Tensor offsets = at::empty({I * tile_w * tile_h}, means2d.options().dtype(at::kInt));
    if (binned_path) {
        Tensor count_ws = bytes(gsx_isect_binned_count_workspace_bytes(rows, uI, utw, uth), means2d);
        { Timed timed_("gsx_isect_binned_count", L.stream); check(gsx_isect_binned_count(fp(means2d), cp<int32_t>(radii), fp(depths), fp(conics), fp(opac), mask_ptr(tile_mask), rows, uI, uts,
                                     utw, uth, mp<int32_t>(tiles_per_gauss), mp<int32_t>(offsets), host_total.mutable_data_ptr<int64_t>(),
                                     host_total.mutable_data_ptr<int64_t>() + 1, count_ws.mutable_data_ptr(), count_ws.numel(), L.stream),
              "gsx_isect_binned_count"); }
        return result(offsets, count_ws, host_total);
    }
    Tensor count_ws = bytes(gsx_isect_fused_count_workspace_bytes(rows, uI, utw, uth), means2d);
    { Timed timed_("gsx_isect_fused_count", L.stream); check(gsx_isect_fused_count(fp(means2d), cp<int32_t>(radii), fp(conics), fp(opac), mask_ptr(tile_mask), rows, uI, uts, utw, uth,
                                mp<int32_t>(tiles_per_gauss), mp<int32_t>(offsets), host_total.mutable_data_ptr<int64_t>(),
                                host_total.mutable_data_ptr<int64_t>() + 1, count_ws.mutable_data_ptr(), count_ws.numel(), L.stream),
          "gsx_isect_fused_count"); }
    return result(offsets, count_ws, host_total);
}

std::tuple<Tensor, Tensor>
isect_fused_finish(const Tensor &means2d, const Tensor &radii, const Tensor &depths, const OptTensor &conics, const OptTensor &opac,
                   const OptTensor &tile_mask, int64_t rows, int64_t I, int64_t tile_size, int64_t tile_w, int64_t tile_h, Tensor count_ws,
                   const Tensor &offsets, const Tensor &host_total, const OptTensor &tiles_per_gauss_)
{
    Tensor tiles_per_gauss = has(tiles_per_gauss_) ? *tiles_per_gauss_ : Tensor();
    Launch L(means2d);
    const uint32_t uI = (uint32_t)I, uts = (uint32_t)tile_size, utw = (uint32_t)tile_w, uth = (uint32_t)tile_h;
    volatile const int64_t *slot = host_total.const_data_ptr<int64_t>();
    auto hip_stream = c10::hip::getCurrentHIPStreamMasqueradingAsCUDA(means2d.device().index());
    int64_t M = poll_host_word(slot, [](int64_t v) { return v == -1; }, hip_stream, std::chrono::seconds(5));
    TORCH_CHECK(host_total.numel() > 2, "isect_fused_finish: host_total must be the three pinned words of isect_fused_begin");
    bool binned = slot[2] != 0;
    if (binned && M == GSX_ISECT_RETRY) {
        binned   = false;
        gsx_isect_binned_note_retry(rows, uI, utw, uth);
        count_ws = bytes(gsx_isect_fused_count_workspace_bytes(rows, uI, utw, uth), means2d);
        { Timed timed_("gsx_isect_fused_count", L.stream); check(gsx_isect_fused_count(fp(means2d), cp<int32_t>(radii), fp(conics), fp(opac), mask_ptr(tile_mask), rows, uI, uts, utw, uth,
                                    mp<int32_t>(tiles_per_gauss), offsets.mutable_data_ptr<int32_t>(),
                                    host_total.mutable_data_ptr<int64_t>(), host_total.mutable_data_ptr<int64_t>() + 1,
                                    count_ws.mutable_data_ptr(), count_ws.numel(), L.stream),
              "gsx_isect_fused_count"); }
        hip_stream.synchronize();
        M = *slot;
    }
    TORCH_CHECK(M >= 0, "intersect_tile: the intersection count never reached the host");
    TORCH_CHECK(M < (1ll << 31), "intersect_tile: ", M, " intersections overflow the int32 index space");
    Tensor ids = at::empty({M}, means2d.options().dtype(at::kLong)), flat = at::empty({M}, means2d.options().dtype(at::kInt));
    if (M == 0) return {ids, flat};
    if (binned) {
        Tensor ws = bytes(gsx_isect_binned_emit_workspace_bytes(M), means2d);
        { Timed timed_("gsx_isect_binned_emit_sort", L.stream); check(gsx_isect_binned_emit_sort(rows, uI, uts, utw, uth, count_ws.mutable_data_ptr(), count_ws.numel(),
                                         cp<int32_t>(offsets), M, (int64_t)slot[1], mp<int64_t>(ids), mp<int32_t>(flat), ws.mutable_data_ptr(), ws.numel(), L.stream),
              "gsx_isect_binned_emit_sort"); }
        note_longest(flat, (int64_t)slot[1]);
        return {ids, flat};
    }
    Tensor ws = bytes(gsx_isect_fused_emit_workspace_bytes(M, uI, utw, uth), means2d);
    { Timed timed_("gsx_isect_fused_emit_sort", L.stream); check(gsx_isect_fused_emit_sort(fp(means2d), cp<int32_t>(radii), fp(depths), fp(conics), fp(opac), mask_ptr(tile_mask), rows, uI, uts,
                                    utw, uth, count_ws.mutable_data_ptr(), count_ws.numel(), cp<int32_t>(offsets), M,
                                    mp<int64_t>(ids), mp<int32_t>(flat), ws.mutable_data_ptr(), ws.numel(), L.stream),
          "gsx_isect_fused_emit_sort"); }
    note_longest(flat, (int64_t)slot[1]);
    return {ids, flat};
}

std::tuple<Tensor, Tensor, Tensor, Tensor, Tensor>
projection_2dgs_fused(const Tensor &means_, const Tensor &quats_, const Tensor &scales_, const Tensor &viewmats_, const Tensor &Ks_,
                      int64_t width, int64_t height, double eps2d, double near_plane, double far_plane, double radius_clip)
{
    (void)eps2d;
    want_f32(means_, "means"); want_f32(quats_, "quats"); want_f32(scales_, "scales"); want_f32(viewmats_, "viewmats");
    want_f32(Ks_, "Ks");
    const int64_t N = means_.size(-2);
    TORCH_CHECK(means_.size(-1) == 3 && quats_.dim() >= 2 && quats_.size(-2) == N && quats_.size(-1) == 4
                          && scales_.dim() >= 2 && scales_.size(-2) == N && scales_.size(-1) == 3,
                      "projection_2dgs: bad shapes means ", means_.sizes(), " quats ", quats_.sizes(), " scales ", scales_.sizes());
    const Tensor means = contig(means_), quats = contig(quats_), scales = contig(scales_), viewmats = contig(viewmats_),
                 Ks = contig(Ks_);
    const int64_t B = prod(means.sizes().slice(0, means.dim() - 2)), C = viewmats.size(-3);
    std::vector<int64_t> shape(means.sizes().begin(), means.sizes().end() - 2);
    shape.push_back(C); shape.push_back(N);
    auto with = [&](std::initializer_list<int64_t> tail) {
        auto s = shape;
        s.insert(s.end(), tail);
        return s;
    };
    Tensor radii = at::empty(with({2}), means.options().dtype(at::kInt)), means2d = at::empty(with({2}), means.options());
    Tensor depths = at::empty(shape, means.options()), rt = at::empty(with({3, 3}), means.options());
    Tensor normals = at::empty(with({3}), means.options());
    if (B * C * N == 0) return {radii, means2d, depths, rt, normals};
    Launch L(means_);
    { Timed timed_("gsx_project_2dgs_fwd", L.stream); check(gsx_project_2dgs_fwd(fp(means), fp(quats), fp(scales), fp(viewmats), fp(Ks), (uint32_t)B, (uint32_t)C, (uint32_t)N,
                               (uint32_t)width, (uint32_t)height, (float)near_plane, (float)far_plane, (float)radius_clip,
                               mp<int32_t>(radii), mp<float>(means2d), mp<float>(depths), mp<float>(rt), mp<float>(normals),
                               L.stream),
          "gsx_project_2dgs_fwd"); }
    return {radii, means2d, depths, rt, normals};
}

std::tuple<Tensor, Tensor, Tensor, Tensor, Tensor, Tensor, Tensor, Tensor>
rasterize_to_pixels_2dgs(const Tensor &means2d_, const Tensor &ray_transforms_, const Tensor &colors_, const Tensor &opacities_,
                         const Tensor &normals_, const Tensor &densify, const OptTensor &backgrounds_, const OptTensor &masks_,
                         int64_t width, int64_t height, int64_t tile_size, const Tensor &tile_offsets_, const Tensor &flatten_ids_,
                         bool packed, bool absgrad, bool distloss)
{
    (void)packed; (void)densify;
    want_f32(means2d_, "means2d"); want_f32(ray_transforms_, "ray_transforms"); want_f32(colors_, "colors");
    want_f32(opacities_, "opacities"); want_f32(normals_, "normals"); want_f32(backgrounds_, "backgrounds");
    Launch L(means2d_);
    const RasterDims r = raster_dims(tile_offsets_, colors_);
    TORCH_CHECK(r.th * tile_size >= height && r.tw * tile_size >= width,
                      "rasterize_to_pixels_2dgs: tile grid does not cover the image");
    TORCH_CHECK(!has(masks_) || masks_->scalar_type() == at::kBool, "masks must be a bool tensor");
    const Tensor means2d = contig(means2d_), rt = contig(ray_transforms_), colors = contig(colors_), opac = contig(opacities_),
                 normals = contig(normals_);
    const OptTensor bg = contig(backgrounds_), masks = contig(masks_);
    const Tensor offsets = contig(tile_offsets_), flat = contig(flatten_ids_);
    auto shape = [&](std::initializer_list<int64_t> tail) {
        auto s = r.image_dims;
        s.insert(s.end(), tail);
        return s;
    };
    const auto f32 = means2d.options(), i32 = means2d.options().dtype(at::kInt);
    Tensor renders = at::empty(shape({height, width, r.D}), f32), alphas = at::empty(shape({height, width, 1}), f32);
    Tensor rnormals = at::empty(shape({height, width, 3}), f32), rdistort = at::empty(shape({height, width, 1}), f32);
    Tensor rmedian = at::empty(shape({height, width, 1}), f32);
    Tensor last_ids = at::empty(shape({height, width}), i32), median_ids = at::empty(shape({height, width}), i32);
    { Timed timed_("gsx_raster2d_fwd", L.stream); check(gsx_raster2d_fwd(fp(means2d), fp(rt), fp(colors), fp(opac), fp(normals), fp(bg),
                           masks ? (const uint8_t *)masks->const_data_ptr<bool>() : nullptr, cp<int32_t>(offsets),
                           cp<int32_t>(flat), (uint32_t)r.I, (uint32_t)flat.numel(), (uint32_t)r.D, (uint32_t)width,
                           (uint32_t)height, (uint32_t)tile_size, (uint32_t)r.tw, (uint32_t)r.th, distloss ? 1 : 0,
                           mp<float>(renders), mp<float>(alphas), mp<float>(rnormals), mp<float>(rdistort), mp<float>(rmedian),
                           mp<int32_t>(last_ids), mp<int32_t>(median_ids), L.stream),
          "gsx_raster2d_fwd"); }
    Tensor holder = absgrad ? at::zeros_like(means2d) : at::empty({0}, f32);
    return {renders, alphas, rnormals, rdistort, rmedian, holder, last_ids, median_ids};
}

}
}

extern "C" int64_t gsx_torch_seg_len() { return gsplat_amd::seg_len_env(); }

TORCH_LIBRARY(gsplat_amd, m)
{
    m.def("isect_fused_begin(Tensor means2d, Tensor radii, Tensor depths, Tensor? conics, Tensor? opacities, Tensor? tile_mask, int rows, int n_images, int tile_size, "
          "int tile_w, int tile_h, int[] out_shape) -> (Tensor?, Tensor, Tensor, Tensor)");
    m.def("isect_fused_finish(Tensor means2d, Tensor radii, Tensor depths, Tensor? conics, Tensor? opacities, Tensor? tile_mask, int rows, int n_images, "
          "int tile_size, int tile_w, int tile_h, Tensor count_ws, Tensor offsets, Tensor host_total, Tensor? tiles_per_gauss) -> (Tensor, Tensor)");
    m.def("note_longest(Tensor flatten_ids, int longest) -> ()");
    m.def("lookup_longest(Tensor flatten_ids) -> int");
    m.def("lookup_seg_workspace(Tensor last_ids, int n_isects, int cdim, int seg_len, Tensor[] inputs) -> Tensor?");
}

TORCH_LIBRARY_IMPL(gsplat_amd, CUDA, m)
{
    m.impl("isect_fused_begin", &gsplat_amd::isect_fused_begin);
    m.impl("isect_fused_finish", &gsplat_amd::isect_fused_finish);
}

TORCH_LIBRARY_IMPL(gsplat_amd, CompositeExplicitAutograd, m)
{
    m.impl("note_longest", &gsplat_amd::note_longest);
    m.impl("lookup_longest", &gsplat_amd::lookup_longest);
    m.impl("lookup_seg_workspace", &gsplat_amd::lookup_seg_workspace);
}

TORCH_LIBRARY_IMPL(gsplat, CUDA, m)
{
    using namespace gsplat_amd;
    m.impl("projection_ewa_3dgs_fused", &projection_ewa_3dgs_fused);
    m.impl("projection_ewa_3dgs_packed", &projection_ewa_3dgs_packed);
    m.impl("intersect_offset", &intersect_offset);
    m.impl("rasterize_to_pixels_3dgs", &rasterize_to_pixels_3dgs);
    m.impl("projection_2dgs_fused", &projection_2dgs_fused);
    m.impl("rasterize_to_pixels_2dgs", &rasterize_to_pixels_2dgs);
}

extern "C" void gsx_torch_profile_begin(const char *only)
{
    using namespace gsplat_amd;
    std::lock_guard<std::mutex> lock(g_prof_mutex);
    g_prof_only.clear();
    std::string w;
    for (const char *p = only ? only : ""; ; ++p) {
        if (*p == ' ' || *p == 0) {
            if (!w.empty()) g_prof_only.insert(w);
            w.clear();
            if (*p == 0) break;
        } else w.push_back(*p);
    }
    g_prof_on = true;
}

extern "C" const char *gsx_torch_profile_end()
{
    using namespace gsplat_amd;
    static std::string out;
    std::lock_guard<std::mutex> lock(g_prof_mutex);
    g_prof_on = false;
    out.clear();
    for (auto &r : g_prof) {
        float ms = 0.0f;
        if (hipEventSynchronize(r.b) == hipSuccess && hipEventElapsedTime(&ms, r.a, r.b) == hipSuccess)
            out += r.name + " " + std::to_string(ms) + "\n";
        (void)hipEventDestroy(r.a);
        (void)hipEventDestroy(r.b);
    }
    g_prof.clear();
    return out.c_str();
}
```

include/gsplat_amd.h:

```cpp
#ifndef GSPLAT_AMD_H_
#define GSPLAT_AMD_H_

#include <stdint.h>

#ifdef __cplusplus
extern "C" {
#endif

#define GSX_ABI_VERSION 1

#define GSX_OK 0
#define GSX_ERR_ARG (-1)
#define GSX_ERR_LAUNCH (-2)
#define GSX_ERR_WORKSPACE (-3)
#define GSX_ERR_OVERFLOW (-4)

#define GSX_CAMERA_PINHOLE 0
#define GSX_CAMERA_ORTHO 1
#define GSX_CAMERA_FISHEYE 2

const char *gsx_last_error(void);
int gsx_version(void);
const char *gsx_arch(void);

// ... 209 lines not shown
                         uint32_t n_images, double fov_horiz_start, double fov_horiz_span, double fov_vert_start,
                         double fov_vert_span, int spinning_ccw, uint32_t n_bins_azimuth, uint32_t n_bins_elevation,
                         uint32_t cdf_resolution_azimuth, uint32_t cdf_resolution_elevation, const int32_t *cdf_elevation,
                         const int32_t *cdf_dense_ray_mask, int64_t *isect_ids, int32_t *flatten_ids, void *stream);

int gsx_project_ut_lidar_fwd(const float *means, const float *quats, const float *scales, const float *opacities,
                             const float *viewmats0, const float *viewmats1, const float *Ks, double fov_horiz_start,
                             double fov_horiz_span, double fov_vert_start, double fov_vert_span, int spinning_ccw,
                             const int32_t *angles_to_columns_map, uint32_t map_h, uint32_t map_w, uint32_t n_columns, uint32_t B,
                             uint32_t C, uint32_t N, float eps2d, float near_plane, float far_plane, float radius_clip,
                             int rs_type, int global_z_order, float ut_alpha, float ut_beta, float ut_kappa,
                             float in_image_margin_factor, int require_all_sigma_points_valid, int32_t *radii, float *means2d,
                             float *depths, float *conics, float *compensations, void *stream);
int gsx_lidar_rays(const float *viewmats, const float *viewmats_rs, const float *row_elevations, const float *column_azimuths,
                   const float *row_azimuth_offsets, uint32_t n_images, uint32_t n_rows, uint32_t n_columns,
                   double fov_horiz_start, double fov_horiz_span, double fov_vert_start, double fov_vert_span, double fov_eps,
                   int spinning_ccw, const int32_t *angles_to_columns_map, uint32_t map_h, uint32_t map_w, int rs_type,
                   float *rays, void *stream);

int gsx_assemble_features_fwd(int degrees_to_use, uint32_t B, uint32_t C, uint32_t N, uint32_t K, uint32_t Dc, uint32_t E,
                              int color_post, int extra_post, int has_depth, int extra_has_c,
                              const float *means, const float *viewmats, const float *coeffs, const float *extra,
                              const float *depths, const uint8_t *masks, float *out, uint8_t *relu_mask, void *stream);

int gsx_sh_band_fwd(int degrees_to_use, int first_band, int coeff_dtype, const float *means, const float *viewmats,
                    const void *coeffs, const uint8_t *masks, const int64_t *batch_ids, const int64_t *camera_ids,
                    const int64_t *gaussian_ids, uint32_t B, uint32_t C, uint32_t N, int64_t nnz, uint32_t K,
                    float *colors, void *stream);
int gsx_sh_band_bwd(int degrees_to_use, int first_band, int coeff_dtype, const float *means, const float *viewmats,
                    const void *coeffs, const uint8_t *masks, uint32_t B, uint32_t C, uint32_t N, int64_t nnz,
                    uint32_t K, const float *v_colors, const int32_t *row_map, void *v_coeffs, float *v_means,
                    float *v_dirs, void *stream);

int gsx_isect_count(const float *means2d, const int32_t *radii, const float *conics, const float *opacities,
                    const int64_t *image_ids, int64_t rows, uint32_t n_per_image, uint32_t n_images,
                    uint32_t tile_size, uint32_t tile_w, uint32_t tile_h, int32_t *tiles_per_gauss, void *stream);
int gsx_isect_emit(const float *means2d, const int32_t *radii, const float *depths, const float *conics,
                   const float *opacities, const int64_t *image_ids, const int64_t *cum_tiles_per_gauss,
                   int64_t rows, uint32_t n_per_image, uint32_t n_images,
                   uint32_t tile_size, uint32_t tile_w, uint32_t tile_h,
                   int64_t *isect_ids, int32_t *flatten_ids, void *stream);
int gsx_isect_count_f64(const double *means2d, const int32_t *radii, const int64_t *image_ids, int64_t rows,
                        uint32_t n_per_image, uint32_t n_images, uint32_t tile_size, uint32_t tile_w, uint32_t tile_h,
                        int32_t *tiles_per_gauss, void *stream);
int gsx_isect_emit_f64(const double *means2d, const int32_t *radii, const double *depths, const int64_t *image_ids,
                       const int64_t *cum_tiles_per_gauss, int64_t rows, uint32_t n_per_image, uint32_t n_images,
                       uint32_t tile_size, uint32_t tile_w, uint32_t tile_h, int64_t *isect_ids, int32_t *flatten_ids,
                       void *stream);
int64_t gsx_scan_workspace_bytes(int64_t n);
int gsx_scan_i32(const int32_t *in, int64_t n, int64_t *out_inclusive, void *workspace, int64_t workspace_bytes,
                 void *stream);
int64_t gsx_sort_pairs_workspace_bytes(int64_t n);
int gsx_sort_pairs(int64_t *keys, int32_t *vals, int64_t *keys_alt, int32_t *vals_alt, int64_t n, int end_bit,
                   void *workspace, int64_t workspace_bytes, int *result_in_alt, void *stream);
int gsx_isect_tile_sort_supported(uint32_t n_images, uint32_t tile_w, uint32_t tile_h);
int64_t gsx_isect_tile_sort_workspace_bytes(int64_t n_isects, uint32_t n_images, uint32_t tile_w, uint32_t tile_h);
int gsx_isect_tile_sort(const int64_t *isect_ids, const int32_t *flatten_ids, int64_t n_isects, uint32_t n_images,
                        uint32_t tile_w, uint32_t tile_h, int64_t *isect_ids_sorted, int32_t *flatten_ids_sorted,
                        void *workspace, int64_t workspace_bytes, void *stream);
int gsx_isect_offsets(const int64_t *isect_ids_sorted, int64_t n_isects, uint32_t n_images, uint32_t tile_w,
                      uint32_t tile_h, int32_t *offsets , void *stream);

int gsx_isect_fused_supported(uint32_t n_images, uint32_t tile_w, uint32_t tile_h, int packed);
int64_t gsx_isect_fused_count_workspace_bytes(int64_t rows, uint32_t n_images, uint32_t tile_w, uint32_t tile_h);
int64_t gsx_isect_fused_emit_workspace_bytes(int64_t n_isects, uint32_t n_images, uint32_t tile_w, uint32_t tile_h);
int gsx_isect_fused_count(const float *means2d, const int32_t *radii, const float *conics, const float *opacities,
                          const uint8_t *tile_mask ,
                          int64_t rows, uint32_t n_images, uint32_t tile_size, uint32_t tile_w, uint32_t tile_h,
                          int32_t *tiles_per_gauss, int32_t *isect_offsets, int64_t *n_isects,
                          int64_t *max_tile_len ,
                          void *count_workspace, int64_t count_workspace_bytes, void *stream);
int gsx_isect_fused_emit_sort(const float *means2d, const int32_t *radii, const float *depths, const float *conics,
                              const float *opacities, const uint8_t *tile_mask, int64_t rows, uint32_t n_images, uint32_t tile_size,
                              uint32_t tile_w, uint32_t tile_h, void *count_workspace, int64_t count_workspace_bytes,
                              const int32_t *isect_offsets, int64_t n_isects, int64_t *isect_ids_sorted,
                              int32_t *flatten_ids_sorted, void *workspace, int64_t workspace_bytes, void *stream);

#define GSX_ISECT_RETRY (-2)
int gsx_isect_binned_supported(int64_t rows, uint32_t n_images, uint32_t tile_w, uint32_t tile_h, int packed);
int gsx_isect_binned_should_try(int64_t rows, uint32_t n_images, uint32_t tile_w, uint32_t tile_h, int packed);
int gsx_isect_binned_note_retry(int64_t rows, uint32_t n_images, uint32_t tile_w, uint32_t tile_h);
void *gsx_isect_path_memory_create(void);
void gsx_isect_path_memory_destroy(void *mem);
void *gsx_isect_path_memory_use(void *mem);
int64_t gsx_isect_binned_count_workspace_bytes(int64_t rows, uint32_t n_images, uint32_t tile_w, uint32_t tile_h);
int64_t gsx_isect_binned_emit_workspace_bytes(int64_t n_isects);
int gsx_isect_binned_count(const float *means2d, const int32_t *radii, const float *depths, const float *conics,
                           const float *opacities, const uint8_t *tile_mask, int64_t rows, uint32_t n_images,
                           uint32_t tile_size, uint32_t tile_w, uint32_t tile_h, int32_t *tiles_per_gauss,
                           int32_t *isect_offsets, int64_t *n_isects, int64_t *max_tile_len ,
                           void *count_workspace, int64_t count_workspace_bytes, void *stream);
int gsx_isect_binned_emit_sort(int64_t rows, uint32_t n_images, uint32_t tile_size, uint32_t tile_w, uint32_t tile_h,
                               void *count_workspace, int64_t count_workspace_bytes, const int32_t *isect_offsets,
                               int64_t n_isects, int64_t longest_list ,
                               int64_t *isect_ids_sorted, int32_t *flatten_ids_sorted, void *workspace,
                               int64_t workspace_bytes, void *stream);

int gsx_raster3d_fwd(const float *means2d, const float *conics, const float *colors, const float *opacities,
                     const float *backgrounds, const uint8_t *masks, const int32_t *isect_offsets,
                     const int32_t *flatten_ids, uint32_t n_images, uint32_t n_isects, uint32_t cdim,
                     uint32_t width, uint32_t height, uint32_t tile_size, uint32_t tile_w, uint32_t tile_h,
                     float *render_colors, float *render_alphas, int32_t *last_ids, void *stream);
int64_t gsx_raster3d_seg_cut(int64_t n_isects, uint32_t n_images, uint32_t tile_w, uint32_t tile_h, uint32_t seg_len);

int64_t gsx_raster3d_seg_workspace_bytes(int64_t n_isects, uint32_t n_images, uint32_t tile_w, uint32_t tile_h, uint32_t cdim,
                                         uint32_t seg_len);
int gsx_raster3d_fwd_seg(const float *means2d, const float *conics, const float *colors, const float *opacities,
                         const float *backgrounds, const uint8_t *masks, const int32_t *isect_offsets,
                         const int32_t *flatten_ids, uint32_t n_images, uint32_t n_isects, uint32_t cdim,
                         uint32_t width, uint32_t height, uint32_t tile_size, uint32_t tile_w, uint32_t tile_h,
                         float *render_colors, float *render_alphas, int32_t *last_ids, uint32_t seg_len, void *workspace,
                         int64_t workspace_bytes, void *stream);
int64_t gsx_raster3d_bwd_seg_workspace_bytes(int64_t n_isects, uint32_t n_images, uint32_t tile_w, uint32_t tile_h, uint32_t cdim,
                                             uint32_t seg_len);
int gsx_raster3d_bwd_seg(const float *means2d, const float *conics, const float *colors, const float *opacities,
                         const float *backgrounds, const uint8_t *masks, const int32_t *isect_offsets,
                         const int32_t *flatten_ids, const float *render_alphas, const int32_t *last_ids,
                         const float *v_render_colors, const float *v_render_alphas, uint32_t n_images, uint32_t n_isects,
                         uint32_t cdim, uint32_t width, uint32_t height, uint32_t tile_size, uint32_t tile_w,
                         uint32_t tile_h, float *v_rows, uint32_t row_stride, uint32_t seg_len, void *workspace,
                         int64_t workspace_bytes, void *stream);
int gsx_raster3d_bwd_seg_reuse(const float *means2d, const float *conics, const float *colors, const float *opacities,
                               const float *backgrounds, const uint8_t *masks, const int32_t *isect_offsets,
                               const int32_t *flatten_ids, const float *render_alphas, const int32_t *last_ids,
                               const float *v_render_colors, const float *v_render_alphas, uint32_t n_images,
                               uint32_t n_isects, uint32_t cdim, uint32_t width, uint32_t height, uint32_t tile_size,
                               uint32_t tile_w, uint32_t tile_h, float *v_rows, uint32_t row_stride, uint32_t seg_len,
                               const void *fwd_workspace, int64_t fwd_workspace_bytes, void *workspace,
                               int64_t workspace_bytes, void *stream);
int gsx_raster3d_bwd(const float *means2d, const float *conics, const float *colors, const float *opacities,
                     const float *backgrounds, const uint8_t *masks, const int32_t *isect_offsets,
                     const int32_t *flatten_ids, const float *render_alphas, const int32_t *last_ids,
                     const float *v_render_colors, const float *v_render_alphas,
                     uint32_t n_images, uint32_t n_isects, uint32_t cdim,
                     uint32_t width, uint32_t height, uint32_t tile_size, uint32_t tile_w, uint32_t tile_h,
                     int has_abs, float *v_rows, uint32_t row_stride, void *stream);
int64_t gsx_raster3d_bwd_workspace_bytes(uint32_t n_images, uint32_t tile_w, uint32_t tile_h);
int gsx_raster3d_bwd_ws(const float *means2d, const float *conics, const float *colors, const float *opacities,
                     const float *backgrounds, const uint8_t *masks, const int32_t *isect_offsets,
                     const int32_t *flatten_ids, const float *render_alphas, const int32_t *last_ids,
                     const float *v_render_colors, const float *v_render_alphas,
                     uint32_t n_images, uint32_t n_isects, uint32_t cdim,
                     uint32_t width, uint32_t height, uint32_t tile_size, uint32_t tile_w, uint32_t tile_h,
                     int has_abs, float *v_rows, uint32_t row_stride, int64_t v_colors_pixel_stride,
                     int64_t v_colors_channel_stride, void *workspace, int64_t workspace_bytes, void *stream);
int gsx_raster3d_bwd_fill(const float *means2d, const float *conics, const float *colors, const float *opacities,
                     const float *backgrounds, const uint8_t *masks, const int32_t *isect_offsets,
                     const int32_t *flatten_ids, const float *render_alphas, const int32_t *last_ids,
                     const float *v_render_colors, const float *v_render_alphas,
                     uint32_t n_images, uint32_t n_isects, uint32_t cdim,
                     uint32_t width, uint32_t height, uint32_t tile_size, uint32_t tile_w, uint32_t tile_h,
                     int has_abs, float *v_rows, uint32_t row_stride, int64_t v_rows_to_fill, int64_t v_colors_pixel_stride,
                     int64_t v_colors_channel_stride, void *workspace, int64_t workspace_bytes, void *stream);

int gsx_raster3d_sparse_fwd(const float *means2d, const float *conics, const float *colors, const float *opacities,
                            const float *backgrounds, const uint8_t *masks, const int32_t *active_tiles,
                            const int32_t *tile_offsets, const int32_t *flatten_ids, const uint64_t *tile_pixel_mask,
                            const int64_t *tile_pixel_cumsum, const int64_t *pixel_map, uint32_t n_active,
                            uint32_t words_per_tile, uint32_t n_images, uint32_t n_isects, uint32_t cdim, uint32_t width,
                            uint32_t height, uint32_t tile_size, uint32_t tile_w, uint32_t tile_h, float *render_colors,
                            float *render_alphas, int32_t *last_ids, void *stream);
int gsx_raster3d_sparse_bwd(const float *means2d, const float *conics, const float *colors, const float *opacities,
                            const float *backgrounds, const uint8_t *masks, const int32_t *active_tiles,
                            const int32_t *tile_offsets, const int32_t *flatten_ids, const uint64_t *tile_pixel_mask,
                            const int64_t *tile_pixel_cumsum, const int64_t *pixel_map, uint32_t n_active,
                            uint32_t words_per_tile, const float *render_alphas, const int32_t *last_ids,
                            const float *v_render_colors, const float *v_render_alphas, uint32_t n_images,
                            uint32_t n_isects, uint32_t cdim, uint32_t width, uint32_t height, uint32_t tile_size,
                            uint32_t tile_w, uint32_t tile_h, int has_abs, float *v_rows, uint32_t row_stride,
                            void *stream);

int gsx_project_simple_fwd(const float *means, const float *covars, const float *Ks, int64_t rows,
                           uint32_t n_per_camera, uint32_t width, uint32_t height, int camera_model, float *means2d,
                           float *covars2d, void *stream);
int gsx_project_simple_bwd(const float *means, const float *covars, const float *Ks, int64_t rows,
                           uint32_t n_per_camera, uint32_t width, uint32_t height, int camera_model,
                           const float *v_means2d, const float *v_covars2d, float *v_means, float *v_covars,
                           void *stream);

int gsx_raster_indices(int mode, uint32_t range_start, uint32_t range_end, const float *transmittances,
                       const float *means2d, const float *geom, const float *opacities, const int32_t *isect_offsets,
                       const int32_t *flatten_ids, uint32_t n_images, uint32_t n_per_image, uint32_t n_isects,
                       uint32_t width, uint32_t height, uint32_t tile_size, uint32_t tile_w, uint32_t tile_h,
                       const int32_t *chunk_starts, int32_t *chunk_cnts, int64_t *gaussian_ids, int64_t *pixel_ids,
                       void *stream);

int gsx_project_2dgs_fwd(const float *means, const float *quats, const float *scales, const float *viewmats,
                         const float *Ks, uint32_t B, uint32_t C, uint32_t N, uint32_t width, uint32_t height,
                         float near_plane, float far_plane, float radius_clip, int32_t *radii, float *means2d,
                         float *depths, float *ray_transforms, float *normals, void *stream);
int gsx_project_2dgs_packed_count(const float *means, const float *quats, const float *scales, const float *viewmats,
                                  const float *Ks, uint32_t B, uint32_t C, uint32_t N, uint32_t width, uint32_t height,
                                  float near_plane, float far_plane, float radius_clip, int32_t *visible, void *stream);
int gsx_project_2dgs_packed_write(const float *means, const float *quats, const float *scales, const float *viewmats,
                                  const float *Ks, uint32_t B, uint32_t C, uint32_t N, uint32_t width, uint32_t height,
                                  float near_plane, float far_plane, float radius_clip, const int64_t *row_offsets,
                                  int64_t nnz, int64_t *batch_ids, int64_t *camera_ids, int64_t *gaussian_ids,
                                  int32_t *indptr, int32_t *radii, float *means2d, float *depths,
                                  float *ray_transforms, float *normals, void *stream);
int gsx_project_2dgs_bwd(const float *means, const float *quats, const float *scales, const float *viewmats,
                         const float *Ks, uint32_t B, uint32_t C, uint32_t N, const int32_t *radii,
                         const float *ray_transforms, const float *v_means2d, const float *v_depths ,
                         const float *v_ray_transforms, const float *v_normals,
                         uint32_t v_row_stride ,
                         uint32_t v_depths_stride ,
                         float *v_means, float *v_quats, float *v_scales, float *v_viewmats, void *stream);
int gsx_project_2dgs_bwd_opac(const float *means, const float *quats, const float *scales, const float *viewmats,
                              const float *Ks, uint32_t B, uint32_t C, uint32_t N, const int32_t *radii,
                              const float *ray_transforms, const float *v_means2d, const float *v_depths,
                              const float *v_ray_transforms, const float *v_normals, uint32_t v_row_stride,
                              uint32_t v_depths_stride, const float *v_view_opacities, uint32_t v_view_opacities_stride, float *v_means,
                              float *v_quats, float *v_scales, float *v_viewmats, float *v_opacities, void *stream);
int gsx_project_2dgs_packed_bwd(const float *means, const float *quats, const float *scales, const float *viewmats,
                                const float *Ks, uint32_t B, uint32_t C, uint32_t N, int64_t nnz,
                                const int64_t *batch_ids, const int64_t *camera_ids, const int64_t *gaussian_ids,
                                const float *ray_transforms, const float *v_means2d, const float *v_depths,
                                const float *v_ray_transforms, const float *v_normals, uint32_t v_row_stride,
                                float *v_means, float *v_quats, float *v_scales, float *v_viewmats, void *stream);
int gsx_project_2dgs_packed_bwd_rows(const float *means, const float *quats, const float *scales, const float *viewmats,
                                     const float *Ks, uint32_t B, uint32_t C, uint32_t N, int64_t nnz,
                                     const int64_t *batch_ids, const int64_t *camera_ids, const int64_t *gaussian_ids,
                                     const float *ray_transforms, const float *v_means2d, const float *v_depths,
                                     const float *v_ray_transforms, const float *v_normals, uint32_t v_row_stride,
                                     float *v_means, float *v_quats, float *v_scales, float *v_viewmats, void *stream);

int gsx_raster2d_fwd(const float *means2d, const float *ray_transforms, const float *colors, const float *opacities,
                     const float *normals, const float *backgrounds, const uint8_t *masks, const int32_t *isect_offsets,
                     const int32_t *flatten_ids, uint32_t n_images, uint32_t n_isects, uint32_t cdim, uint32_t width,
                     uint32_t height, uint32_t tile_size, uint32_t tile_w, uint32_t tile_h, int distloss,
                     float *render_colors, float *render_alphas, float *render_normals, float *render_distort,
                     float *render_median, int32_t *last_ids, int32_t *median_ids, void *stream);
int gsx_raster2d_bwd(const float *means2d, const float *ray_transforms, const float *colors, const float *opacities,
                     const float *normals, const float *backgrounds, const uint8_t *masks, const int32_t *isect_offsets,
                     const int32_t *flatten_ids, const float *render_colors, const float *render_alphas,
                     const int32_t *last_ids, const int32_t *median_ids, const float *v_render_colors,
                     const float *v_render_alphas, const float *v_render_normals, const float *v_render_distort,
                     const float *v_render_median, uint32_t n_images, uint32_t n_isects, uint32_t cdim, uint32_t width,
                     uint32_t height, uint32_t tile_size, uint32_t tile_w, uint32_t tile_h, int has_abs, float *v_rows,
                     uint32_t row_stride, void *stream);
int gsx_raster2d_bwd_ws(const float *means2d, const float *ray_transforms, const float *colors, const float *opacities,
                     const float *normals, const float *backgrounds, const uint8_t *masks, const int32_t *isect_offsets,
                     const int32_t *flatten_ids, const float *render_colors, const float *render_alphas,
                     const int32_t *last_ids, const int32_t *median_ids, const float *v_render_colors,
                     const float *v_render_alphas, const float *v_render_normals, const float *v_render_distort,
                     const float *v_render_median, uint32_t n_images, uint32_t n_isects, uint32_t cdim, uint32_t width,
                     uint32_t height, uint32_t tile_size, uint32_t tile_w, uint32_t tile_h, int has_abs, float *v_rows,
                     uint32_t row_stride, void *workspace, int64_t workspace_bytes, void *stream);
int gsx_raster2d_bwd_fill(const float *means2d, const float *ray_transforms, const float *colors, const float *opacities,
                     const float *normals, const float *backgrounds, const uint8_t *masks, const int32_t *isect_offsets,
                     const int32_t *flatten_ids, const float *render_colors, const float *render_alphas,
                     const int32_t *last_ids, const int32_t *median_ids, const float *v_render_colors,
                     const float *v_render_alphas, const float *v_render_normals, const float *v_render_distort,
                     const float *v_render_median, uint32_t n_images, uint32_t n_isects, uint32_t cdim, uint32_t width,
                     uint32_t height, uint32_t tile_size, uint32_t tile_w, uint32_t tile_h, int has_abs, float *v_rows,
                     uint32_t row_stride, int64_t v_rows_to_fill, void *workspace, int64_t workspace_bytes, void *stream);

int gsx_surfel_post_fwd(const float *colors, const float *alphas, const float *normals, const float *median,
                        const float *viewmats, const float *Ks, uint32_t n_images, uint32_t width, uint32_t height,
                        uint32_t cdim, int expected_depth, int depth_source, float *colors_out, float *normals_world,
                        float *surf_normals, void *stream);
int gsx_surfel_post_bwd(const float *colors, const float *alphas, const float *normals, const float *median,
                        const float *viewmats, const float *Ks, uint32_t n_images, uint32_t width, uint32_t height,
                        uint32_t cdim, int expected_depth, int depth_source, const float *v_colors_out,
                        const float *v_normals_world, const float *v_surf_normals, float *v_colors, float *v_alphas,
                        float *v_normals, float *v_median, void *stream);

int gsx_raster3d_pair_stats(const float *means2d, const float *conics, const float *opacities,
                            const int32_t *isect_offsets, const int32_t *flatten_ids, uint32_t n_images,
                            uint32_t n_isects, uint32_t width, uint32_t height, uint32_t tile_size, uint32_t tile_w,
                            uint32_t tile_h, uint64_t *stats, void *stream);

int gsx_raster3d_num_contributing(const float *means2d, const float *conics, const float *opacities,
                                  const int32_t *isect_offsets, const int32_t *flatten_ids, uint32_t n_images,
                                  uint32_t n_isects, uint32_t n_per_image, uint32_t width, uint32_t height,
                                  uint32_t tile_size, uint32_t tile_w, uint32_t tile_h, int32_t *counts, float *alphas,
                                  void *stream);
int gsx_raster3d_contributing_ids(const float *means2d, const float *conics, const float *opacities,
                                  const int32_t *isect_offsets, const int32_t *flatten_ids, uint32_t n_images,
                                  uint32_t n_isects, uint32_t n_per_image, uint32_t width, uint32_t height,
                                  uint32_t tile_size, uint32_t tile_w, uint32_t tile_h, uint32_t max_contributing,
                                  int32_t *ids, float *weights, void *stream);
int gsx_raster3d_top_contributing(const float *means2d, const float *conics, const float *opacities,
                                  const int32_t *isect_offsets, const int32_t *flatten_ids, uint32_t n_images,
                                  uint32_t n_isects, uint32_t n_per_image, uint32_t width, uint32_t height,
                                  uint32_t tile_size, uint32_t tile_w, uint32_t tile_h, uint32_t num_depth_samples,
                                  int32_t *ids, float *weights, void *stream);

int gsx_raster3d_sparse_num_contributing(const float *means2d, const float *conics, const float *opacities,
        const int32_t *active_tiles, const int32_t *tile_offsets, const int32_t *flatten_ids,
        const uint64_t *tile_pixel_mask, const int64_t *tile_pixel_cumsum, const int64_t *pixel_map,
        uint32_t n_active, uint32_t words_per_tile, uint32_t n_images, uint32_t n_isects, uint32_t n_per_image,
        uint32_t width, uint32_t height, uint32_t tile_size, uint32_t tile_w, uint32_t tile_h, int32_t *counts, float *alphas, void *stream);
int gsx_raster3d_sparse_contributing_ids(const float *means2d, const float *conics, const float *opacities,
        const int32_t *active_tiles, const int32_t *tile_offsets, const int32_t *flatten_ids,
        const uint64_t *tile_pixel_mask, const int64_t *tile_pixel_cumsum, const int64_t *pixel_map,
        uint32_t n_active, uint32_t words_per_tile, uint32_t n_images, uint32_t n_isects, uint32_t n_per_image,
        uint32_t width, uint32_t height, uint32_t tile_size, uint32_t tile_w, uint32_t tile_h, uint32_t max_contributing, int32_t *ids, float *weights,
        void *stream);
int gsx_raster3d_sparse_top_contributing(const float *means2d, const float *conics, const float *opacities,
        const int32_t *active_tiles, const int32_t *tile_offsets, const int32_t *flatten_ids,
        const uint64_t *tile_pixel_mask, const int64_t *tile_pixel_cumsum, const int64_t *pixel_map,
        uint32_t n_active, uint32_t words_per_tile, uint32_t n_images, uint32_t n_isects, uint32_t n_per_image,
        uint32_t width, uint32_t height, uint32_t tile_size, uint32_t tile_w, uint32_t tile_h, uint32_t num_depth_samples, int32_t *ids, float *weights,
        void *stream);

int gsx_copy_column_groups(uint32_t n_groups, const void *const *src, const uint32_t *src_strides, void *const *dst,
// ... 111 lines not shown
```

Before: 2450 Mpixels/s.

## Emit per-tile cost from forward raster to skip backward cost pass

The forward rasterizer now computes each tile's work (last contributing index minus range start) with a block-wide max reduction and writes it to a tile_cost tensor, which is saved for backward. The backward tile-order builder can then use these precomputed costs instead of rereading last_ids in its own cost kernel, which is meant to cut the cost-kernel memory traffic. In exchange the forward pass gains an extra reduction, a __syncthreads and a small tensor, and there is a new autograd forward path plus op registration.

```diff
diff --git a/gsplat_amd/_autograd.py b/gsplat_amd/_autograd.py
--- a/gsplat_amd/_autograd.py
+++ b/gsplat_amd/_autograd.py
@@ -167,7 +167,7 @@
                                v_row_opacities)
 
 
-def _rast_setup(ctx, inputs, output):
+def _rast_setup(ctx, inputs, output, tile_cost=None):
     (means2d, conics, colors, opacities, backgrounds, masks, image_width, image_height, tile_size, isect_offsets,
      flatten_ids, _packed, absgrad) = inputs
     _render_colors, render_alphas, means2d_absgrad, last_ids = output
@@ -177,16 +177,27 @@
     ctx.rc_shape = _render_colors.shape
     ctx.longest = _ops._lookup_longest(flatten_ids)
     ctx.save_for_backward(means2d, conics, colors, opacities, backgrounds, masks, isect_offsets, flatten_ids,
-                          render_alphas, last_ids, means2d_absgrad)
+                          render_alphas, last_ids, means2d_absgrad, tile_cost)
+
+
+def _rast_forward(ctx, *args):
+    *out, tile_cost = _rast_cost_op(*args)
+    out = tuple(out)
+    _rast_setup(ctx, args, out, tile_cost if tile_cost.numel() else None)
+    return out
+
+
+_rast_cost_op = torch.ops.gsplat_amd.rasterize_to_pixels_3dgs_cost.default
 
 
 def _rast_backward(ctx, v_render_colors, v_render_alphas, v_means2d_absgrad, v_last_ids):
     (means2d, conics, colors, opacities, backgrounds, masks, isect_offsets, flatten_ids, render_alphas, last_ids,
-     means2d_absgrad) = ctx.saved_tensors
+     means2d_absgrad, tile_cost) = ctx.saved_tensors
     v_means2d_abs, v_means2d, v_conics, v_colors, v_opacities, v_backgrounds = _bwd("rasterize_to_pixels_3dgs")(
         means2d, conics, colors, opacities, backgrounds, masks, isect_offsets, flatten_ids, render_alphas, last_ids,
         ctx.width, ctx.height, ctx.tile_size, ctx.absgrad, _z(v_render_colors, ctx.rc_shape, render_alphas),
         None if v_render_alphas is None else v_render_alphas.contiguous(), ctx.needs_input_grad[4], _longest=ctx.longest,
+        _tile_cost=tile_cost,
     )
     if ctx.absgrad and v_means2d_abs is not None:
         means2d_absgrad.copy_(v_means2d_abs)
@@ -377,6 +388,9 @@
 register()
 
 
+_FORWARD = {"rasterize_to_pixels_3dgs": _rast_forward}
+
+
 class _FastOps:
 
     def __init__(self, extra=None):
@@ -393,11 +407,14 @@
         else:
             bwd, setup = entry
             overload = op.default
+            own_forward = _FORWARD.get(name)
 
             class _Fn(torch.autograd.Function):
                 @staticmethod
                 def forward(ctx, *args):
                     with torch._C._AutoDispatchBelowAutograd():
+                        if own_forward is not None:
+                            return own_forward(ctx, *args)
                         out = overload(*args)
                     setup(ctx, args, out)
                     return out
diff --git a/gsplat_amd/_cabi.py b/gsplat_amd/_cabi.py
--- a/gsplat_amd/_cabi.py
+++ b/gsplat_amd/_cabi.py
@@ -202,19 +202,19 @@
     return out
 
 
-def call(name: str, *args) -> None:
+def call(name: str, *args, label: Optional[str] = None) -> None:
     dev = getattr(_tls, "dev", None)
     if dev is not None and dev != torch.cuda.current_device():
         _tls.dev = None
         with torch.cuda.device(dev):
-            return call(name, *args)
+            return call(name, *args, label=label)
     fn = getattr(_lib, name)
-    if _profile is not None and (_profile_only is None or name in _profile_only):
+    if _profile is not None and (_profile_only is None or (label or name) in _profile_only):
         a, b = torch.cuda.Event(enable_timing=True), torch.cuda.Event(enable_timing=True)
         a.record()
         rc = fn(*args, current_stream())
         b.record()
-        _profile.append((name, a, b))
+        _profile.append((label or name, a, b))
     else:
         rc = fn(*args, current_stream())
     if rc != 0:
diff --git a/gsplat_amd/_ops.py b/gsplat_amd/_ops.py
--- a/gsplat_amd/_ops.py
+++ b/gsplat_amd/_ops.py
@@ -754,7 +754,7 @@
 @_op("rasterize_to_pixels_3dgs_bwd")
 def rasterize_to_pixels_3dgs_bwd(means2d, conics, colors, opacities, backgrounds, masks, tile_offsets, flatten_ids,
                                  render_alphas, last_ids, image_width, image_height, tile_size, absgrad,
-                                 v_render_colors, v_render_alphas, compute_v_backgrounds, *, _longest=None):
+                                 v_render_colors, v_render_alphas, compute_v_backgrounds, *, _longest=None, _tile_cost=None):
     image_dims, I, th, tw, D = _raster_dims(tile_offsets, colors)
     as_received = (means2d, conics, colors, opacities, tile_offsets, flatten_ids)
     means2d, conics, colors, opacities = (means2d.contiguous(), conics.contiguous(), colors.contiguous(),
@@ -782,11 +782,13 @@
              0 if fws is None else fws.numel(), ptr(ws), ws.numel())
     else:
         ws = torch.empty(_cabi._lib.gsx_raster3d_bwd_workspace_bytes(I, tw, th), device=means2d.device, dtype=torch.uint8)
-        call("gsx_raster3d_bwd_fill", ptr(means2d), ptr(conics), ptr(colors), ptr(opacities), ptr(backgrounds), ptr(masks),
+        if _tile_cost is not None and (_tile_cost.numel() != I * tw * th or _tile_cost.dtype != torch.int32):
+            _tile_cost = None
+        call("gsx_raster3d_bwd_cost", ptr(means2d), ptr(conics), ptr(colors), ptr(opacities), ptr(backgrounds), ptr(masks),
              ptr(tile_offsets.contiguous()), ptr(flatten_ids.contiguous()), ptr(render_alphas.contiguous()),
-             ptr(last_ids.contiguous()), ptr_strided(v_render_colors), ptr(v_render_alphas), I, flatten_ids.numel(), D,
-             image_width, image_height, tile_size, tw, th, int(bool(absgrad)), ptr(rows), geo + D, R, vrc_strides[0],
-             vrc_strides[1], ptr(ws), ws.numel())
+             ptr(last_ids.contiguous()), ptr(_tile_cost), ptr_strided(v_render_colors), ptr(v_render_alphas), I,
+             flatten_ids.numel(), D, image_width, image_height, tile_size, tw, th, int(bool(absgrad)), ptr(rows), geo + D, R,
+             vrc_strides[0], vrc_strides[1], ptr(ws), ws.numel(), label="gsx_raster3d_bwd_fill")
     v_means2d, v_conics = rows[:, 0:2].view(means2d.shape), rows[:, 2:5].view(conics.shape)
     v_opacities, v_colors = rows[:, 5].view(opacities.shape), rows[:, geo:].view(colors.shape)
     v_abs = rows[:, 6:8].view(means2d.shape) if absgrad else None
diff --git a/gsplat_amd/csrc/raster3d.hpp b/gsplat_amd/csrc/raster3d.hpp
--- a/gsplat_amd/csrc/raster3d.hpp
+++ b/gsplat_amd/csrc/raster3d.hpp
@@ -47,6 +47,7 @@
     float *seg_out;
     int32_t *seg_last;
     const int32_t *tile_order;
+    int32_t *tile_cost;
 };
 
 inline Raster3DArgs raster3d_args(uint32_t n_images, uint32_t n_isects, uint32_t cdim, uint32_t width, uint32_t height,
@@ -191,7 +192,8 @@
 int64_t tile_order_workspace_bytes(uint32_t n_images, uint32_t tile_w, uint32_t tile_h);
 const int32_t *build_tile_order(const int32_t *isect_offsets, const int32_t *last_ids, uint32_t n_images, uint32_t tile_size,
                                 uint32_t tile_w, uint32_t tile_h, uint32_t width, uint32_t height, uint32_t n_isects, void *ws,
-                                int64_t ws_bytes, hipStream_t stream, int *rc, void *zero_ptr = nullptr, int64_t zero_bytes = 0);
+                                int64_t ws_bytes, hipStream_t stream, int *rc, void *zero_ptr = nullptr, int64_t zero_bytes = 0,
+                                const int32_t *tile_cost = nullptr);
 
 struct RowFill {
     const char *fn;
@@ -199,11 +201,12 @@
     int64_t bytes;
     hipStream_t stream;
     template <class Args>
-    const int32_t *tile_order(const Args &a, void *ws, int64_t ws_bytes, int *rc)
+    const int32_t *tile_order(const Args &a, void *ws, int64_t ws_bytes, int *rc, const int32_t *tile_cost = nullptr)
     {
         const bool in_kernel = bytes > 0 && (reinterpret_cast<uintptr_t>(rows) & 15u) == 0;
         const int32_t *order = build_tile_order(a.isect_offsets, a.last_ids, a.n_images, a.tile_size, a.tile_w, a.tile_h, a.width,
-                                                a.height, a.n_isects, ws, ws_bytes, stream, rc, in_kernel ? rows : nullptr, bytes);
+                                                a.height, a.n_isects, ws, ws_bytes, stream, rc, in_kernel ? rows : nullptr, bytes,
+                                                tile_cost);
         if (*rc == GSX_OK && order && in_kernel) bytes = 0;
         return order;
     }
diff --git a/gsplat_amd/csrc/raster3d_bwd.hip b/gsplat_amd/csrc/raster3d_bwd.hip
--- a/gsplat_amd/csrc/raster3d_bwd.hip
+++ b/gsplat_amd/csrc/raster3d_bwd.hip
@@ -1003,6 +1003,20 @@
     uint32_t tile_w, uint32_t tile_h, int has_abs, float *v_rows, uint32_t row_stride, int64_t v_rows_to_fill,
     int64_t v_colors_pixel_stride, int64_t v_colors_channel_stride, void *workspace, int64_t workspace_bytes, void *stream)
 {
+    return gsx_raster3d_bwd_cost(means2d, conics, colors, opacities, backgrounds, masks, isect_offsets, flatten_ids, render_alphas,
+                                 last_ids, nullptr, v_render_colors, v_render_alphas, n_images, n_isects, cdim, width, height,
+                                 tile_size, tile_w, tile_h, has_abs, v_rows, row_stride, v_rows_to_fill, v_colors_pixel_stride,
+                                 v_colors_channel_stride, workspace, workspace_bytes, stream);
+}
+
+extern "C" int gsx_raster3d_bwd_cost(
+    const float *means2d, const float *conics, const float *colors, const float *opacities,
+    const float *backgrounds, const uint8_t *masks, const int32_t *isect_offsets, const int32_t *flatten_ids,
+    const float *render_alphas, const int32_t *last_ids, const int32_t *tile_cost, const float *v_render_colors,
+    const float *v_render_alphas, uint32_t n_images, uint32_t n_isects, uint32_t cdim, uint32_t width, uint32_t height,
+    uint32_t tile_size, uint32_t tile_w, uint32_t tile_h, int has_abs, float *v_rows, uint32_t row_stride, int64_t v_rows_to_fill,
+    int64_t v_colors_pixel_stride, int64_t v_colors_channel_stride, void *workspace, int64_t workspace_bytes, void *stream)
+{
     using namespace gsx;
     RowFill fill{"gsx_raster3d_bwd_fill", v_rows, v_rows_to_fill > 0 ? v_rows_to_fill * (int64_t)row_stride * 4 : 0,
                  (hipStream_t)stream};
@@ -1024,7 +1038,7 @@
     }
     if (raster3d_bwd_kernel(tile_size, cdim > 32 ? 32 : cdim, has_abs != 0) != BwdKernel::R) {
         int rc       = GSX_OK;
-        a.tile_order = fill.tile_order(a, workspace, workspace_bytes, &rc);
+        a.tile_order = fill.tile_order(a, workspace, workspace_bytes, &rc, tile_cost);
         if (rc != GSX_OK) return rc;
     }
     if (int rc = fill.now(); rc != GSX_OK) return rc;
diff --git a/gsplat_amd/csrc/raster3d_fwd.hip b/gsplat_amd/csrc/raster3d_fwd.hip
--- a/gsplat_amd/csrc/raster3d_fwd.hip
+++ b/gsplat_amd/csrc/raster3d_fwd.hip
@@ -33,6 +33,7 @@
     const size_t pix = inside ? (size_t)prow : 0;
 
     const float *bg = a.backgrounds ? a.backgrounds + (size_t)image_id * a.cdim + a.ch_off : nullptr;
+    __shared__ int32_t s_m[4];
 
     if (a.masks && !a.masks[(size_t)image_id * tiles_per_image + tile_id]) {
         if constexpr (PRE) {
@@ -59,6 +60,8 @@
                 a.last_ids[pix]      = 0;
             }
         }
+        if (a.tile_cost && tid == 0)
+            a.tile_cost[(size_t)image_id * tiles_per_image + tile_id] = max(0, min(tc.range_end, 1) - tc.range_start);
         return;
     }
 
@@ -67,7 +70,6 @@
     int32_t last_id   = -1;
     if constexpr (PRE) {
         last_id = inside ? a.last_ids[pix] : -1;
-        __shared__ int32_t s_m[4];
         const int32_t wm = wave_max_i32(last_id);
         if ((tid & 63u) == 0) s_m[tid >> 6] = wm;
         __syncthreads();
@@ -183,6 +185,15 @@
         a.seg_last[(size_t)seg_item * 256 + tid] = (int32_t)cur_idx;
         return;
     }
+    if (a.tile_cost) {
+        const int32_t wm = wave_max_i32(inside ? (int32_t)cur_idx : -1);
+        if (lane == 0) s_m[tid >> 6] = wm;
+        __syncthreads();
+        if (tid == 0) {
+            const int32_t m = max(max(s_m[0], s_m[1]), max(s_m[2], s_m[3]));
+            a.tile_cost[(size_t)image_id * tiles_per_image + tile_id] = max(0, min(range_end, m + 1) - range_start);
+        }
+    }
     if (inside) {
 #pragma unroll
         for (int k = 0; k < CH; ++k)
@@ -224,10 +235,17 @@
     return with_channels(a.nch, [&](auto ch) { return launch_fwd<ch()>(a, stream); });
 }
 
+static bool raster3d_fwd_emits_cost(Raster3DArgs a)
+{
+    a.nch = a.cdim > 32 ? 32 : a.cdim;
+    return a.tile_size == 16 && !a.sp_active_tiles && a.seg_mode == 0 && a.seg_len == 0 && !raster3d_fwd_m_applies(a);
+}
+
 int raster3d_fwd_dispatch(Raster3DArgs a, hipStream_t stream)
 {
     uint32_t off = 0;
     bool first   = true;
+    if (!raster3d_fwd_emits_cost(a)) a.tile_cost = nullptr;
     do {
         const uint32_t rem = a.cdim - off;
         const uint32_t n   = rem > 32 ? 32 : rem;
@@ -238,6 +256,7 @@
         if (rc != GSX_OK) return rc;
         off += n;
         first = false;
+        a.tile_cost = nullptr;
     } while (off < a.cdim);
     return GSX_OK;
 }
@@ -249,6 +268,25 @@
     const float *backgrounds, const uint8_t *masks, const int32_t *isect_offsets, const int32_t *flatten_ids,
     uint32_t n_images, uint32_t n_isects, uint32_t cdim, uint32_t width, uint32_t height, uint32_t tile_size,
     uint32_t tile_w, uint32_t tile_h, float *render_colors, float *render_alphas, int32_t *last_ids, void *stream)
+{
+    return gsx_raster3d_fwd_cost(means2d, conics, colors, opacities, backgrounds, masks, isect_offsets, flatten_ids, n_images,
+                                 n_isects, cdim, width, height, tile_size, tile_w, tile_h, render_colors, render_alphas, last_ids,
+                                 nullptr, stream);
+}
+
+extern "C" int gsx_raster3d_fwd_emits_cost(uint32_t tile_size, uint32_t cdim)
+{
+    gsx::Raster3DArgs a{};
+    a.tile_size = tile_size; a.cdim = cdim;
+    return cdim >= 1 && gsx::raster3d_fwd_emits_cost(a) ? 1 : 0;
+}
+
+extern "C" int gsx_raster3d_fwd_cost(
+    const float *means2d, const float *conics, const float *colors, const float *opacities,
+    const float *backgrounds, const uint8_t *masks, const int32_t *isect_offsets, const int32_t *flatten_ids,
+    uint32_t n_images, uint32_t n_isects, uint32_t cdim, uint32_t width, uint32_t height, uint32_t tile_size,
+    uint32_t tile_w, uint32_t tile_h, float *render_colors, float *render_alphas, int32_t *last_ids, int32_t *tile_cost,
+    void *stream)
 {
     using namespace gsx;
     GSX_REQUIRE(tile_size >= 1 && tile_size <= 16, "gsx_raster3d_fwd: tile_size must be in [1,16], got %u", tile_size);
@@ -259,6 +297,9 @@
     GSX_REQUIRE(isect_offsets != nullptr || n_images * tile_w * tile_h == 0, "gsx_raster3d_fwd: null isect_offsets");
     Raster3DArgs a = raster3d_args(n_images, n_isects, cdim, width, height, tile_size, tile_w, tile_h, means2d, conics, colors,
                                    opacities, backgrounds, masks, isect_offsets, flatten_ids, render_colors, render_alphas, last_ids);
+    GSX_REQUIRE(!tile_cost || raster3d_fwd_emits_cost(a),
+                "gsx_raster3d_fwd_cost: no tile costs from tile_size %u with %u channels (gsx_raster3d_fwd_emits_cost)", tile_size, cdim);
+    a.tile_cost = tile_cost;
     return raster3d_fwd_dispatch(a, (hipStream_t)stream);
 }
 
diff --git a/gsplat_amd/csrc/tile_order.hip b/gsplat_amd/csrc/tile_order.hip
--- a/gsplat_amd/csrc/tile_order.hip
+++ b/gsplat_amd/csrc/tile_order.hip
@@ -1,6 +1,7 @@
 #include <cstdlib>
 
 #include "raster3d.hpp"
+#include "../../include/gsplat_amd.h"
 
 namespace gsx {
 
@@ -9,19 +10,24 @@
     const int32_t *isect_offsets, *last_ids;
     uint32_t n_images, tile_w, tile_h, width, height, n_isects, n_blocks, per_xcd;
     int32_t *cost;
+    const int32_t *cost_in;
+    uint32_t n_sort;
     int32_t *order;
     void *zero_ptr;
     int64_t zero_bytes;
 };
+template <uint32_t THREADS>
+__device__ __forceinline__ void tile_order_fill(const TileOrderArgs &a, uint32_t block, uint32_t n_blocks)
+{
+    const int64_t n16 = a.zero_bytes >> 4;
+    uint4 *z          = reinterpret_cast<uint4 *>(a.zero_ptr);
+    for (int64_t i = (int64_t)block * THREADS + threadIdx.x; i < n16; i += (int64_t)n_blocks * THREADS) z[i] = make_uint4(0u, 0u, 0u, 0u);
+    if (block == 0 && (int64_t)threadIdx.x < ((a.zero_bytes & 15) >> 2))
+        reinterpret_cast<float *>(a.zero_ptr)[n16 * 4 + threadIdx.x] = 0.0f;
+}
 __global__ void __launch_bounds__(256) tile_order_cost_kernel(const TileOrderArgs a)
 {
-    if (a.zero_ptr) {
-        const int64_t n16 = a.zero_bytes >> 4;
-        uint4 *z          = reinterpret_cast<uint4 *>(a.zero_ptr);
-        for (int64_t i = (int64_t)blockIdx.x * 256 + threadIdx.x; i < n16; i += (int64_t)gridDim.x * 256) z[i] = make_uint4(0u, 0u, 0u, 0u);
-        if (blockIdx.x == 0 && (int64_t)threadIdx.x < ((a.zero_bytes & 15) >> 2))
-            reinterpret_cast<float *>(a.zero_ptr)[n16 * 4 + threadIdx.x] = 0.0f;
-    }
+    if (a.zero_ptr) tile_order_fill<256>(a, blockIdx.x, gridDim.x);
     const uint32_t lane = threadIdx.x & 63u, blk = blockIdx.x * 4u + (threadIdx.x >> 6);
     if (blk >= a.n_blocks) return;
     const uint32_t tiles_per_image = a.tile_w * a.tile_h;
@@ -40,16 +46,16 @@
         a.cost[blk]         = max(0, min(end, m + 1) - start);
     }
 }
-__global__ void __launch_bounds__(1024) tile_order_sort_kernel(const TileOrderArgs a)
+__device__ __forceinline__ void tile_order_sort_range(const TileOrderArgs &a, uint32_t range)
 {
     __shared__ int32_t s_hist[kOrderBuckets];
     __shared__ int32_t s_wave[16];
     const uint32_t tid = threadIdx.x, lane = tid & 63u, wave = tid >> 6;
-    const uint32_t first = blockIdx.x * a.per_xcd, last = min(first + a.per_xcd, a.n_blocks);
+    const uint32_t first = range * a.per_xcd, last = min(first + a.per_xcd, a.n_blocks);
     s_hist[tid] = 0;
     __syncthreads();
     for (uint32_t blk = first + tid; blk < last; blk += 1024u)
-        atomicAdd(&s_hist[min((uint32_t)a.cost[blk] >> 2, kOrderBuckets - 1u)], 1);
+        atomicAdd(&s_hist[min((uint32_t)a.cost_in[blk] >> 2, kOrderBuckets - 1u)], 1);
     __syncthreads();
     const int32_t mine = s_hist[kOrderBuckets - 1u - tid];
     int32_t inc        = mine;
@@ -65,9 +71,15 @@
     s_hist[kOrderBuckets - 1u - tid] = before + inc - mine;
     __syncthreads();
     for (uint32_t blk = first + tid; blk < last; blk += 1024u) {
-        const int32_t slot = atomicAdd(&s_hist[min((uint32_t)a.cost[blk] >> 2, kOrderBuckets - 1u)], 1);
+        const int32_t slot = atomicAdd(&s_hist[min((uint32_t)a.cost_in[blk] >> 2, kOrderBuckets - 1u)], 1);
         a.order[first + (uint32_t)slot] = (int32_t)blk;
     }
+}
+__global__ void __launch_bounds__(1024) tile_order_sort_kernel(const TileOrderArgs a) { tile_order_sort_range(a, blockIdx.x); }
+__global__ void __launch_bounds__(1024) tile_order_sort_fill_kernel(const TileOrderArgs a)
+{
+    if (blockIdx.x < a.n_sort) tile_order_sort_range(a, blockIdx.x);
+    else tile_order_fill<1024>(a, blockIdx.x - a.n_sort, gridDim.x - a.n_sort);
 }
 
 }
@@ -86,12 +98,13 @@
 }
 const int32_t *build_tile_order(const int32_t *isect_offsets, const int32_t *last_ids, uint32_t n_images, uint32_t tile_size,
                                 uint32_t tile_w, uint32_t tile_h, uint32_t width, uint32_t height, uint32_t n_isects, void *ws,
-                                int64_t ws_bytes, hipStream_t stream, int *rc, void *zero_ptr, int64_t zero_bytes)
+                                int64_t ws_bytes, hipStream_t stream, int *rc, void *zero_ptr, int64_t zero_bytes,
+                                const int32_t *tile_cost)
 {
     *rc = GSX_OK;
     const uint32_t n_blocks = tile_w * tile_h * n_images;
     const int mode = bwd_lpt_mode();
-    if (!ws || tile_size != 16 || mode == 0 || (mode == 1 && n_blocks < 2048u)) return nullptr;
+    if (!ws || tile_size != 16 || n_blocks == 0 || mode == 0 || (mode == 1 && n_blocks < 2048u)) return nullptr;
     if (ws_bytes < tile_order_workspace_bytes(n_images, tile_w, tile_h)) return nullptr;
     TileOrderArgs o{};
     o.isect_offsets = isect_offsets; o.last_ids = last_ids; o.n_images = n_images; o.tile_w = tile_w; o.tile_h = tile_h;
@@ -99,8 +112,16 @@
     o.cost  = reinterpret_cast<int32_t *>(ws);
     o.order = o.cost + n_blocks;
     o.zero_ptr = zero_ptr; o.zero_bytes = zero_bytes;
-    tile_order_cost_kernel<<<dim3((n_blocks + 3u) / 4u), dim3(256), 0, stream>>>(o);
-    tile_order_sort_kernel<<<dim3((n_blocks + o.per_xcd - 1u) / o.per_xcd), dim3(1024), 0, stream>>>(o);
+    o.cost_in = tile_cost ? tile_cost : o.cost;
+    o.n_sort  = (n_blocks + o.per_xcd - 1u) / o.per_xcd;
+    if (tile_cost && zero_ptr) {
+        const int64_t per_block = 1024 * 4 * 16;
+        const int64_t n_fill    = (zero_bytes + per_block - 1) / per_block;
+        tile_order_sort_fill_kernel<<<dim3(o.n_sort + (uint32_t)(n_fill < 1 ? 1 : n_fill > 2048 ? 2048 : n_fill)), dim3(1024), 0, stream>>>(o);
+    } else {
+        if (!tile_cost) tile_order_cost_kernel<<<dim3((n_blocks + 3u) / 4u), dim3(256), 0, stream>>>(o);
+        tile_order_sort_kernel<<<dim3(o.n_sort), dim3(1024), 0, stream>>>(o);
+    }
     *rc = check_launch("tile order");
     return *rc == GSX_OK ? o.order : nullptr;
 }
@@ -112,3 +133,20 @@
 }
 
 }
+
+extern "C" int gsx_raster3d_tile_order(const int32_t *isect_offsets, const int32_t *last_ids, const int32_t *tile_cost,
+                                       uint32_t n_images, uint32_t tile_size, uint32_t tile_w, uint32_t tile_h, uint32_t width,
+                                       uint32_t height, uint32_t n_isects, void *workspace, int64_t workspace_bytes,
+                                       void *zero_ptr, int64_t zero_bytes, void *stream)
+{
+    using namespace gsx;
+    GSX_REQUIRE(isect_offsets && (last_ids || tile_cost), "gsx_raster3d_tile_order: null input");
+    GSX_REQUIRE(!zero_ptr || ((reinterpret_cast<uintptr_t>(zero_ptr) & 15u) == 0 && zero_bytes >= 0 && (zero_bytes & 3) == 0),
+                "gsx_raster3d_tile_order: zero_ptr must be 16-byte aligned and zero_bytes a multiple of 4");
+    int rc = GSX_OK;
+    const int32_t *order = build_tile_order(isect_offsets, last_ids, n_images, tile_size, tile_w, tile_h, width, height, n_isects,
+                                            workspace, workspace_bytes, (hipStream_t)stream, &rc, zero_ptr, zero_bytes, tile_cost);
+    if (rc != GSX_OK) return rc;
+    GSX_REQUIRE(order, "gsx_raster3d_tile_order: no order for this launch (tile size, workspace, tile count or GSX_RASTER3D_BWD_ORDER)");
+    return GSX_OK;
+}
diff --git a/gsplat_amd/csrc/torch_ops.cpp b/gsplat_amd/csrc/torch_ops.cpp
--- a/gsplat_amd/csrc/torch_ops.cpp
+++ b/gsplat_amd/csrc/torch_ops.cpp
@@ -375,9 +375,9 @@
 #define kSegLen (seg_len_env())
 
 std::tuple<Tensor, Tensor, Tensor, Tensor>
-rasterize_to_pixels_3dgs(const Tensor &means2d_, const Tensor &conics_, const Tensor &colors_, const Tensor &opacities_,
-                         const OptTensor &backgrounds_, const OptTensor &masks_, int64_t width, int64_t height, int64_t tile_size,
-                         const Tensor &isect_offsets_, const Tensor &flatten_ids_, bool packed, bool absgrad)
+raster3d_fwd_body(const Tensor &means2d_, const Tensor &conics_, const Tensor &colors_, const Tensor &opacities_,
+                  const OptTensor &backgrounds_, const OptTensor &masks_, int64_t width, int64_t height, int64_t tile_size,
+                  const Tensor &isect_offsets_, const Tensor &flatten_ids_, bool packed, bool absgrad, Tensor *tile_cost)
 {
     (void)packed;
     want_f32(means2d_, "means2d"); want_f32(conics_, "conics"); want_f32(colors_, "colors"); want_f32(opacities_, "opacities");
@@ -411,14 +411,40 @@
               "gsx_raster3d_fwd_seg");
         if (r.D <= 4 && tile_size == 16 && seg_reuse_env())
             note_seg_workspace(last_ids, ws, flat.numel(), r.D, kSegLen, {means2d_, conics_, colors_, opacities_, isect_offsets_, flatten_ids_});
-    } else { Timed timed_("gsx_raster3d_fwd", L.stream); check(gsx_raster3d_fwd(fp(means2d), fp(conics), fp(colors), fp(opac), fp(bg),
+    } else {
+        Tensor cost;
+        if (tile_cost && gsx_raster3d_fwd_emits_cost((uint32_t)tile_size, (uint32_t)r.D))
+            cost = at::empty({r.I * r.th * r.tw}, means2d.options().dtype(at::kInt));
+        Timed timed_("gsx_raster3d_fwd", L.stream); check(gsx_raster3d_fwd_cost(fp(means2d), fp(conics), fp(colors), fp(opac), fp(bg),
                            masks ? (const uint8_t *)masks->const_data_ptr<bool>() : nullptr, cp<int32_t>(offsets),
                            cp<int32_t>(flat), (uint32_t)r.I, (uint32_t)flat.numel(), (uint32_t)r.D, (uint32_t)width,
                            (uint32_t)height, (uint32_t)tile_size, (uint32_t)r.tw, (uint32_t)r.th, mp<float>(renders),
-                           mp<float>(alphas), mp<int32_t>(last_ids), L.stream),
-          "gsx_raster3d_fwd"); }
+                           mp<float>(alphas), mp<int32_t>(last_ids), mp<int32_t>(cost), L.stream),
+          "gsx_raster3d_fwd");
+        if (cost.defined()) *tile_cost = cost;
+    }
     Tensor holder = absgrad ? at::zeros_like(means2d) : at::empty({0}, means2d.options());
     return {renders, alphas, holder, last_ids};
+}
+
+std::tuple<Tensor, Tensor, Tensor, Tensor>
+rasterize_to_pixels_3dgs(const Tensor &means2d, const Tensor &conics, const Tensor &colors, const Tensor &opacities,
+                         const OptTensor &backgrounds, const OptTensor &masks, int64_t width, int64_t height, int64_t tile_size,
+                         const Tensor &isect_offsets, const Tensor &flatten_ids, bool packed, bool absgrad)
+{
+    return raster3d_fwd_body(means2d, conics, colors, opacities, backgrounds, masks, width, height, tile_size, isect_offsets,
+                             flatten_ids, packed, absgrad, nullptr);
+}
+
+std::tuple<Tensor, Tensor, Tensor, Tensor, Tensor>
+rasterize_to_pixels_3dgs_cost(const Tensor &means2d, const Tensor &conics, const Tensor &colors, const Tensor &opacities,
+                              const OptTensor &backgrounds, const OptTensor &masks, int64_t width, int64_t height,
+                              int64_t tile_size, const Tensor &isect_offsets, const Tensor &flatten_ids, bool packed, bool absgrad)
+{
+    Tensor tile_cost = at::empty({0}, isect_offsets.options().dtype(at::kInt));
+    auto [renders, alphas, holder, last_ids] = raster3d_fwd_body(means2d, conics, colors, opacities, backgrounds, masks, width, height,
+                                                                 tile_size, isect_offsets, flatten_ids, packed, absgrad, &tile_cost);
+    return {renders, alphas, holder, last_ids, tile_cost};
 }
 
 const uint8_t *mask_ptr(const OptTensor &m) { return has(m) && m->numel() ? (const uint8_t *)m->const_data_ptr<bool>() : nullptr; }
@@ -592,12 +618,16 @@
     m.def("note_longest(Tensor flatten_ids, int longest) -> ()");
     m.def("lookup_longest(Tensor flatten_ids) -> int");
     m.def("lookup_seg_workspace(Tensor last_ids, int n_isects, int cdim, int seg_len, Tensor[] inputs) -> Tensor?");
+    m.def("rasterize_to_pixels_3dgs_cost(Tensor means2d, Tensor conics, Tensor colors, Tensor opacities, Tensor? backgrounds, Tensor? masks, "
+          "int image_width, int image_height, int tile_size, Tensor isect_offsets, Tensor flatten_ids, bool packed, bool absgrad) "
+          "-> (Tensor, Tensor, Tensor, Tensor, Tensor)");
 }
 
 TORCH_LIBRARY_IMPL(gsplat_amd, CUDA, m)
 {
     m.impl("isect_fused_begin", &gsplat_amd::isect_fused_begin);
     m.impl("isect_fused_finish", &gsplat_amd::isect_fused_finish);
+    m.impl("rasterize_to_pixels_3dgs_cost", &gsplat_amd::rasterize_to_pixels_3dgs_cost);
 }
 
 TORCH_LIBRARY_IMPL(gsplat_amd, CompositeExplicitAutograd, m)
diff --git a/include/gsplat_amd.h b/include/gsplat_amd.h
--- a/include/gsplat_amd.h
+++ b/include/gsplat_amd.h
@@ -385,6 +385,24 @@
                      uint32_t width, uint32_t height, uint32_t tile_size, uint32_t tile_w, uint32_t tile_h,
                      int has_abs, float *v_rows, uint32_t row_stride, int64_t v_rows_to_fill, int64_t v_colors_pixel_stride,
                      int64_t v_colors_channel_stride, void *workspace, int64_t workspace_bytes, void *stream);
+int gsx_raster3d_fwd_emits_cost(uint32_t tile_size, uint32_t cdim);
+int gsx_raster3d_fwd_cost(const float *means2d, const float *conics, const float *colors, const float *opacities,
+                          const float *backgrounds, const uint8_t *masks, const int32_t *isect_offsets,
+                          const int32_t *flatten_ids, uint32_t n_images, uint32_t n_isects, uint32_t cdim,
+                          uint32_t width, uint32_t height, uint32_t tile_size, uint32_t tile_w, uint32_t tile_h,
+                          float *render_colors, float *render_alphas, int32_t *last_ids, int32_t *tile_cost, void *stream);
+int gsx_raster3d_bwd_cost(const float *means2d, const float *conics, const float *colors, const float *opacities,
+                          const float *backgrounds, const uint8_t *masks, const int32_t *isect_offsets,
+                          const int32_t *flatten_ids, const float *render_alphas, const int32_t *last_ids,
+                          const int32_t *tile_cost, const float *v_render_colors, const float *v_render_alphas,
+                          uint32_t n_images, uint32_t n_isects, uint32_t cdim,
+                          uint32_t width, uint32_t height, uint32_t tile_size, uint32_t tile_w, uint32_t tile_h,
+                          int has_abs, float *v_rows, uint32_t row_stride, int64_t v_rows_to_fill, int64_t v_colors_pixel_stride,
+                          int64_t v_colors_channel_stride, void *workspace, int64_t workspace_bytes, void *stream);
+int gsx_raster3d_tile_order(const int32_t *isect_offsets, const int32_t *last_ids, const int32_t *tile_cost,
+                            uint32_t n_images, uint32_t tile_size, uint32_t tile_w, uint32_t tile_h, uint32_t width,
+                            uint32_t height, uint32_t n_isects, void *workspace, int64_t workspace_bytes, void *zero_ptr,
+                            int64_t zero_bytes, void *stream);
 
 int gsx_raster3d_sparse_fwd(const float *means2d, const float *conics, const float *colors, const float *opacities,
                             const float *backgrounds, const uint8_t *masks, const int32_t *active_tiles,
```

Result: no change. 2461 Mpixels/s, median of 6 (+0.5%).
